# UCL/gp_emulator

Hardware: AMD Instinct MI355X
Metric: test-points/sec for predict(mean+var+grad), N_train=250 D=11 (higher is better)
Workload: dtype f64

## Files before the change

gp_emulator_amd/_lib.py:

```python
import ctypes
import os
import sys
import threading

import numpy as np

from ._dense_numpy import (DAMPINGS, newton_step_numpy, posterior_cov_numpy, prec_rows, prior_propagate_numpy,
                           prior_rows, row_strides, rts_smooth_numpy, _cholesky_inverse_numpy, _mirror_lower)
from ._lut_numpy import MAX_PCS as lut_pc_max_pcs
from ._lut_numpy import lut_pc_prepare_numpy, lut_search_numpy, lut_search_pc_numpy
from ._moments_numpy import rows_arrays as _moments_rows
from ._sobol_numpy import bounds_arrays as _sobol_bounds

HERE = os.path.dirname(os.path.abspath(__file__))
LIB_PATH = os.environ.get("GP_PREDICT_LIB") or os.path.join(HERE, "libgp_predict_hip.so")

GP_F32, GP_F64 = 0, 1
GP_DERIV_DMAJOR, GP_DERIV_ROWMAJOR = 0, 1
GP_DAMP_DIAGONAL, GP_DAMP_IDENTITY = 0, 1
_DAMPING = dict(zip(DAMPINGS, (GP_DAMP_DIAGONAL, GP_DAMP_IDENTITY)))

c_int, c_i64, c_void_p = ctypes.c_int, ctypes.c_int64, ctypes.c_void_p
c_dp = ctypes.POINTER(ctypes.c_double)
c_fp = ctypes.POINTER(ctypes.c_float)
PP = ctypes.POINTER(c_void_p)

SIGNATURES = {
    "gp_last_error_string": (ctypes.c_char_p, []),
    "gp_version_string": (ctypes.c_char_p, []),
    "gp_device_count": (c_int, [ctypes.POINTER(c_int)]),
    "gp_ctx_create": (c_int, [c_int, PP]),
    "gp_ctx_destroy": (c_int, [c_void_p]),
    "gp_ctx_synchronize": (c_int, [c_void_p]),
    "gp_ctx_set_debug_buffer": (c_int, [c_void_p, c_void_p]),
    "gp_ctx_device_info": (c_int, [c_void_p, ctypes.POINTER(c_int), ctypes.POINTER(c_i64),
                                   ctypes.c_char_p, c_int]),
    "gp_predict_wrap_f64": (c_int, [c_void_p] + [c_void_p] * 8 + [c_i64, c_int, c_int, c_int]),
    "gp_predict_wrap_f32": (c_int, [c_void_p] + [c_void_p] * 8 + [c_i64, c_int, c_int, c_int]),
    "gp_predict_rows_f64": (c_int, [c_void_p] + [c_void_p] * 8 + [c_i64, c_int, c_int, c_int]),
    "gp_predict_rows_f32": (c_int, [c_void_p] + [c_void_p] * 8 + [c_i64, c_int, c_int, c_int]),
    "gp_predict_rows_f32_h64": (c_int, [c_void_p] + [c_void_p] * 8 + [c_i64, c_int, c_int, c_int]),
    "gp_model_create_f64": (c_int, [c_void_p] + [c_void_p] * 4 + [c_int, c_int, c_int, PP]),
    "gp_model_create_f32": (c_int, [c_void_p] + [c_void_p] * 4 + [c_int, c_int, c_int, PP]),
    "gp_model_create_f32_h64": (c_int, [c_void_p] + [c_void_p] * 4 + [c_int, c_int, c_int, PP]),
    "gp_batch_create_f32_h64": (c_int, [c_void_p, c_int] + [c_void_p] * 4 + [c_int, c_int, c_int, PP]),
    "gp_batch_create_f64": (c_int, [c_void_p, c_int] + [c_void_p] * 4 + [c_int, c_int, c_int, PP]),
    "gp_batch_create_f32": (c_int, [c_void_p, c_int] + [c_void_p] * 4 + [c_int, c_int, c_int, PP]),
    "gp_model_emulators": (c_int, [c_void_p, ctypes.POINTER(c_int)]),
    "gp_model_destroy": (c_int, [c_void_p]),
    "gp_model_info": (c_int, [c_void_p] + [ctypes.POINTER(c_int)] * 5),
    "gp_predict_device": (c_int, [c_void_p, c_void_p, c_void_p, c_void_p, c_void_p, c_void_p,
                                  c_i64, c_int]),
    "gp_predict_host": (c_int, [c_void_p, c_void_p, c_int, c_void_p, c_void_p, c_void_p, c_void_p,
                                c_i64, c_int, c_i64]),
    "gp_predict_mean_grad_device": (c_int, [c_void_p, c_void_p, c_void_p, c_void_p, c_void_p, c_i64, c_int]),
    "gp_predict_var_grad_device": (c_int, [c_void_p, c_void_p, c_void_p, c_void_p, c_void_p, c_i64, c_int]),
    "gp_model_var_grad_bytes": (c_int, [c_void_p, ctypes.POINTER(c_i64)]),
    "gp_predict_mean_grad_host": (c_int, [c_void_p, c_void_p, c_int, c_void_p, c_void_p, c_void_p,
                                          c_i64, c_int, c_i64]),
    "gp_ctx_host_threads": (c_int, [c_void_p, ctypes.POINTER(c_int)]),
    "gp_device_numa_node": (c_int, [c_int, ctypes.POINTER(c_int)]),
    "gp_kernel_ksteps": (c_int, [c_int, c_int, ctypes.POINTER(c_int)]),
    "gp_hessian_device": (c_int, [c_void_p, c_void_p, c_void_p, c_void_p, c_i64]),
    "gp_hessian_host": (c_int, [c_void_p, c_void_p, c_void_p, c_void_p, c_i64]),
    "gp_hessian_weighted_device": (c_int, [c_void_p, c_void_p, c_void_p, c_void_p, c_void_p, c_i64]),
    "gp_hessian_weighted_host": (c_int, [c_void_p, c_void_p, c_int, c_void_p, c_void_p, c_void_p, c_i64]),
    "gp_band_misfit_device": (c_int, [c_void_p, c_void_p, c_void_p, c_void_p, c_i64, c_i64, c_void_p, c_i64, c_i64,
                                      c_void_p, c_void_p, c_void_p, c_void_p, c_void_p, c_i64]),
    "gp_band_misfit_unc_device": (c_int, [c_void_p, c_void_p, c_void_p, c_void_p, c_i64, c_i64, c_void_p, c_i64, c_i64,
                                          c_void_p, c_void_p, c_void_p, c_void_p, c_void_p, c_i64]),
    "gp_band_misfit_host": (c_int, [c_void_p, c_void_p, c_int, c_void_p, c_void_p, c_i64, c_i64, c_void_p, c_i64, c_i64,
                                    c_void_p, c_void_p, c_void_p, c_void_p, c_void_p, c_i64]),
    "gp_newton_step_device": (c_int, [c_void_p, c_int] + [c_void_p] * 4 + [c_int] + [c_void_p] * 7 + [c_i64, c_int]),
    "gp_lm_update_device": (c_int, [c_void_p, c_int] + [c_void_p] * 14 + [ctypes.c_double] * 6 + [c_i64, c_int]),
    "gp_posterior_cov_device": (c_int, [c_void_p, c_int] + [c_void_p] * 5 + [c_i64, c_int]),
    "gp_newton_step_rows_device": (c_int, [c_void_p, c_int] + [c_void_p] * 4 + [c_int] + [c_void_p] * 7 + [c_i64, c_int, c_i64, c_i64]),
    "gp_lm_update_rows_device": (c_int, [c_void_p, c_int] + [c_void_p] * 14 + [ctypes.c_double] * 6 + [c_i64, c_int, c_i64, c_i64]),
    "gp_posterior_cov_rows_device": (c_int, [c_void_p, c_int] + [c_void_p] * 5 + [c_i64, c_int, c_i64]),
    "gp_prior_propagate_device": (c_int, [c_void_p, c_int, c_void_p, c_void_p, c_i64, c_void_p, c_i64, c_void_p, c_void_p, c_i64, c_int]),
    "gp_rts_smooth_device": (c_int, [c_void_p, c_int, c_void_p, c_void_p, c_i64, c_void_p, c_i64] + [c_void_p] * 9 + [c_i64, c_int]),
    "gp_lut_search_device": (c_int, [c_void_p, c_int, c_void_p, c_i64, c_i64, c_void_p, c_void_p, c_i64, c_i64, c_void_p,
                                     c_i64, c_i64, c_void_p, c_void_p, c_i64, c_i64, c_int, c_int, c_int]),
    "gp_lut_search_geometry": (c_int, [ctypes.POINTER(c_int)] * 3),
    "gp_lut_search_pc_device": (c_int, [c_void_p, c_int, c_void_p, c_i64, c_i64] + [c_void_p] * 5 + [c_i64] + [c_void_p] * 3
                                + [c_i64, c_i64, c_int, c_int, c_int]),
    "gp_lut_search_pc_geometry": (c_int, [c_int, c_int] + [ctypes.POINTER(c_int)] * 4),
    "gp_mv_lut_prepare_device": (c_int, [c_void_p, c_int, c_void_p, c_void_p, c_i64, c_void_p, c_i64, c_void_p, c_i64]
                                 + [c_void_p] * 4 + [c_i64, c_int, c_int]),
    "gp_hessian_f64": (c_int, [c_void_p] + [c_void_p] * 5 + [c_i64, c_int, c_int, c_int]),
    "gp_hessian_f32": (c_int, [c_void_p] + [c_void_p] * 5 + [c_i64, c_int, c_int, c_int]),
    "gp_reconstruct_device": (c_int, [c_void_p, c_int, c_void_p, c_void_p, c_void_p, c_i64, c_int, c_int]),
    "gp_hessian_host_h64": (c_int, [c_void_p, c_void_p, c_void_p, c_void_p, c_i64]),
    "gp_mv_predict_host": (c_int, [c_void_p, c_void_p, c_void_p, c_void_p, c_i64, c_int, c_void_p, c_void_p]),
    "gp_content_digest": (ctypes.c_uint64, [c_void_p, c_void_p, c_int]),
    "gp_mv_predict_host_checked": (c_int, [c_void_p, c_void_p, c_void_p, c_void_p, c_i64, c_int, c_void_p, c_void_p,
                                           c_void_p, c_void_p, c_int, ctypes.c_uint64]),
    "gp_mv_misfit_device": (c_int, [c_void_p, c_int, c_void_p, c_void_p, c_void_p, c_void_p, c_i64, c_void_p, c_i64,
                                    c_void_p, c_void_p, c_void_p, c_i64, c_int, c_int, c_int]),
    "gp_mv_gauss_newton_device": (c_int, [c_void_p, c_int, c_void_p, c_void_p, c_void_p, c_i64, c_int, c_int]),
    "gp_mv_weight_gram_device": (c_int, [c_void_p, c_int, c_void_p, c_void_p, c_i64, c_void_p, c_i64, c_int, c_int]),
    "gp_mv_gauss_newton_rows_device": (c_int, [c_void_p, c_int, c_void_p, c_void_p, c_i64, c_void_p, c_i64, c_int, c_int]),
    "gp_mv_misfit_unc_device": (c_int, [c_void_p, c_int, c_void_p, c_void_p, c_void_p, c_i64] + [c_void_p] * 8
                                + [c_i64, c_int, c_int]),
    "gp_mv_misfit_host": (c_int, [c_void_p, c_void_p, c_void_p, c_void_p, c_i64, c_void_p, c_i64, c_void_p, c_i64,
                                  c_void_p, c_i64, c_int, c_void_p]),
    "gp_mv_misfit_host_checked": (c_int, [c_void_p, c_void_p, c_void_p, c_void_p, c_i64, c_void_p, c_i64, c_void_p, c_i64,
                                          c_void_p, c_i64, c_int, c_void_p, c_void_p, c_void_p, c_int, ctypes.c_uint64]),
    "gp_frag_index": (c_int, [c_int, c_int, c_int, c_int]),
    "gp_likelihood_batch_f64": (c_int, [c_void_p, c_int, c_void_p, c_void_p, c_void_p, c_int, c_int,
                                        c_int, c_void_p, c_void_p, c_void_p, c_void_p]),
    "gp_sobol_batch_f64": (c_int, [c_void_p, c_int, c_void_p, c_void_p, c_void_p, c_int, c_int, c_int, c_void_p, c_void_p,
                                   c_int, c_void_p, c_void_p, c_void_p]),
    "gp_moments_batch_f64": (c_int, [c_void_p, c_int, c_void_p, c_void_p, c_void_p, c_void_p, c_int, c_int, c_i64, c_void_p,
                                     c_void_p, c_int, c_void_p, c_void_p, c_void_p, c_void_p, c_void_p, c_void_p]),
    "gp_pack_sizes": (c_int, [c_int, c_int, c_int, ctypes.POINTER(c_int), ctypes.POINTER(c_int),
                              ctypes.POINTER(c_i64), ctypes.POINTER(c_i64)]),
    "gp_launch_plan": (c_int, [c_int, c_int, c_int, c_int, c_int, c_i64, c_int, c_int, c_int, ctypes.POINTER(c_int),
                               ctypes.POINTER(c_i64), ctypes.POINTER(c_int), ctypes.POINTER(c_i64),
                               ctypes.POINTER(c_int), ctypes.POINTER(c_int)]),
    "gp_pack_model_f64": (c_int, [c_void_p] * 4 + [c_int, c_int, c_int] + [c_void_p] * 4),
    "gp_pack_model_f32": (c_int, [c_void_p] * 4 + [c_int, c_int, c_int] + [c_void_p] * 4),
    "gp_pinned_alloc": (c_int, [c_void_p, c_i64, PP]),
    "gp_pinned_free": (c_int, [c_void_p, c_void_p]),
    "gp_malloc": (c_int, [c_void_p, c_i64, PP]),
    "gp_free": (c_int, [c_void_p, c_void_p]),
    "gp_memcpy_h2d": (c_int, [c_void_p, c_void_p, c_void_p, c_i64]),
    "gp_memcpy_d2h": (c_int, [c_void_p, c_void_p, c_void_p, c_i64]),
    "gp_memset": (c_int, [c_void_p, c_void_p, c_int, c_i64]),
    "gp_event_create": (c_int, [c_void_p, PP]),
    "gp_event_destroy": (c_int, [c_void_p]),
    "gp_event_record": (c_int, [c_void_p, c_void_p]),
    "gp_event_elapsed_ms": (c_int, [c_void_p, c_void_p, ctypes.POINTER(ctypes.c_float)]),
}


class GpuPredictUnavailable(RuntimeError):
    """The HIP library is missing or unusable.  Never caught inside this package."""


class GpuPredictError(RuntimeError):
    """A C-ABI call returned a non-zero status."""


_lib = None
_lock = threading.Lock()


def load():
    global _lib
    with _lock:
        if _lib is not None:
            return _lib
        if not os.path.exists(LIB_PATH):
            raise GpuPredictUnavailable(
                "%s not built; run `python -m gp_emulator_amd.build` (needs hipcc). "
                "There is no CPU fallback for is_gpu=True." % LIB_PATH)
        try:
            lib = ctypes.CDLL(LIB_PATH)
        except OSError as e:
            raise GpuPredictUnavailable("cannot load %s: %s" % (LIB_PATH, e))
        for name, (res, args) in SIGNATURES.items():
            fn = getattr(lib, name)
            fn.restype = res
            fn.argtypes = args
        _lib = lib
        return lib


def check(rc, what=""):
    if rc != 0:
        msg = load().gp_last_error_string().decode("utf-8", "replace")
        raise GpuPredictError("%s failed (status %d): %s" % (what or "gp call", rc, msg))


GP_STALE = 1


class HostBlocks:

    def __init__(self, arrays):
        self.arrays = list(arrays)
        self.ids = tuple(id(a) for a in arrays)
        self._bufs = {}
        src = []
        for i, a in enumerate(self.arrays):
            if isinstance(a, np.ndarray) and a.flags.c_contiguous:
                src.append(a)
            else:
                self._bufs[i] = np.array(a, order="C", copy=True)
                src.append(self._bufs[i])
        self.n = len(src)
        self.ptrs = (c_void_p * self.n)(*[a.ctypes.data for a in src])
        self.lens = (c_i64 * self.n)(*[a.nbytes for a in src])
        self.expected = self.digest()

    def same_arrays(self, arrays):
        return self.ids == tuple(id(a) for a in arrays)

    def refresh(self):
        for i, buf in self._bufs.items():
            a = np.asarray(self.arrays[i])
            if a.shape == buf.shape and a.dtype == buf.dtype:
                np.copyto(buf, a)
            else:
                buf.view(np.uint8)[...] = 0xA5
        return self

    def digest(self):
        self.refresh()
        return int(load().gp_content_digest(self.ptrs, self.lens, self.n))

    def unchanged(self):
        return self.digest() == self.expected


def device_count():
    n = c_int(0)
    rc = load().gp_device_count(ctypes.byref(n))
    if rc != 0:
        return 0
    return n.value


def _ptr(a):
    return a.ctypes.data_as(c_void_p)


def _dtype_code(dtype):
    return GP_F64 if np.dtype(dtype) == np.float64 else GP_F32


def precision_dtype(precision):
    dt = np.dtype(precision)
    if dt not in (np.dtype(np.float32), np.dtype(np.float64)):
        raise TypeError("precision must be float32 or float64, got %r" % (precision,))
    return dt


def _out_array(a, shape, dtype, pool=None):
    if a is None:
        return pool.take(shape, dtype) if pool is not None else np.empty(shape, dtype)
    if (not isinstance(a, np.ndarray) or a.dtype != dtype or a.shape != shape
            or not a.flags["C_CONTIGUOUS"] or not a.flags["WRITEABLE"]):
        raise ValueError("out must be a writeable C-contiguous %s %s array" % (shape, np.dtype(dtype)))
    return a


def _device_dtype(precision, a):
    return np.dtype(precision if precision is not None else (np.float32 if a.dtype == np.float32 else np.float64))


def _matrix_rows(A, precision):
    A = np.asarray(A)
    if A.ndim != 3 or A.shape[1] != A.shape[2]:
        raise ValueError("A must be (n_rows, n_inputs, n_inputs)")
    return A, _device_dtype(precision, A), A.shape[0], A.shape[1]


def device_numa_cpus(device=0):
    node = c_int(-1)
    if load().gp_device_numa_node(int(device), ctypes.byref(node)) != 0 or node.value < 0:
        return set()
    try:
        text = open("/sys/devices/system/node/node%d/cpulist" % node.value).read().strip()
    except OSError:
        return set()
    cpus = set()
    for part in text.split(","):
        if part:
            a, _, b = part.partition("-")
            cpus.update(range(int(a), int(b or a) + 1))
    return cpus & set(os.sched_getaffinity(0))


def bind_near_device(device=0):
    cpus = device_numa_cpus(device)
    if cpus:
        os.sched_setaffinity(0, cpus)
    return cpus


class OutputPool:

    def __init__(self, max_item=256 << 20, max_total=1 << 30):
        self.max_item, self.max_total = max_item, max_total
        self.items = []

    def take(self, shape, dtype):
        dtype = np.dtype(dtype)
        nbytes = int(np.prod(shape, dtype=np.int64)) * dtype.itemsize
        if nbytes < (1 << 20) or nbytes > self.max_item:
            return np.empty(shape, dtype)
        base = None
        for cand in self.items:
            if cand.nbytes == nbytes and sys.getrefcount(cand) == 3:
                base = cand
                break
        cand = None
        if base is None:
            base = np.empty(nbytes, np.uint8)
            self.items.append(base)
            total = sum(b.nbytes for b in self.items)
            for free_first in (True, False):
                i = 0
                while total > self.max_total and i < len(self.items):
                    b = self.items[i]
                    if b is not base and (not free_first or sys.getrefcount(b) == 3):
                        total -= b.nbytes
                        del self.items[i]
                    else:
                        i += 1
                b = None
        return base.view(dtype).reshape(shape)


class Scratch(object):

    def __init__(self, ctx, dt):
        self.ctx, self.dt, self.held = ctx, dt, []

    def up(self, a):
        if a is None:
            return None
        self.held.append(self.ctx.to_device(np.ascontiguousarray(a, dtype=self.dt)))
        return self.held[-1]

    def alloc(self, nbytes):
        self.held.append(self.ctx.malloc(max(1, nbytes)))
        return self.held[-1]

    def __enter__(self):
        return self

    def __exit__(self, *exc):
        held, self.held = self.held, []
        for p in held:
            self.ctx.free(p)


def _download(ctx, dptr, shape, dtype):
    return np.array(ctx.to_host(dptr, shape, dtype))


class Context:

    def __init__(self, device=0):
        self.lib = load()
        h = c_void_p()
        rc = self.lib.gp_ctx_create(int(device), ctypes.byref(h))
        if rc != 0:
            msg = self.lib.gp_last_error_string().decode("utf-8", "replace")
            raise GpuPredictUnavailable("no usable GPU context on device %d: %s" % (device, msg))
        self.h = h
        self.device = int(device)
        self.out_pool = OutputPool()

    def pinned_empty(self, shape, dtype=np.float64):
        import weakref
        dtype = np.dtype(dtype)
        n = int(np.prod(shape, dtype=np.int64))
        nbytes = max(1, n * dtype.itemsize)
        ptr = c_void_p()
        check(self.lib.gp_pinned_alloc(self.h, nbytes, ctypes.byref(ptr)), "gp_pinned_alloc")
        buf = (ctypes.c_char * nbytes).from_address(ptr.value)
        arr = np.frombuffer(buf, dtype=np.uint8, count=n * dtype.itemsize).view(dtype).reshape(shape)
        lib, h, addr = self.lib, self.h, ptr.value
        weakref.finalize(buf, lambda: lib.gp_pinned_free(h, c_void_p(addr)))
        return arr

    def close(self):
        if getattr(self, "h", None):
            self.lib.gp_ctx_destroy(self.h)
            self.h = None

    __del__ = close

    def synchronize(self):
        check(self.lib.gp_ctx_synchronize(self.h), "gp_ctx_synchronize")

    def device_info(self):
        cu, mem = c_int(0), c_i64(0)
        name = ctypes.create_string_buffer(256)
        check(self.lib.gp_ctx_device_info(self.h, ctypes.byref(cu), ctypes.byref(mem), name, 256))
        return dict(compute_units=cu.value, hbm_bytes=mem.value, name=name.value.decode())

    def host_threads(self):
        n = c_int(0)
        check(self.lib.gp_ctx_host_threads(self.h, ctypes.byref(n)), "gp_ctx_host_threads")
        return n.value

    def malloc(self, nbytes):
        p = c_void_p()
        check(self.lib.gp_malloc(self.h, int(nbytes), ctypes.byref(p)), "gp_malloc")
        return p

    def free(self, p):
        check(self.lib.gp_free(self.h, p), "gp_free")

    def to_device(self, arr):
        arr = np.ascontiguousarray(arr)
        p = self.malloc(max(arr.nbytes, 1))
        if arr.nbytes:
            check(self.lib.gp_memcpy_h2d(self.h, p, _ptr(arr), arr.nbytes), "gp_memcpy_h2d")
        return p

    def h2d(self, dptr, arr):
        arr = np.ascontiguousarray(arr)
        check(self.lib.gp_memcpy_h2d(self.h, dptr, _ptr(arr), arr.nbytes), "gp_memcpy_h2d")

    def to_host(self, dptr, shape, dtype):
        out = self.out_pool.take(shape, dtype)
        if out.nbytes:
            check(self.lib.gp_memcpy_d2h(self.h, _ptr(out), dptr, out.nbytes), "gp_memcpy_d2h")
        return out

    def to_host_at(self, dptr, offset_bytes, shape, dtype):
        out = np.empty(shape, dtype=dtype)
        src = c_void_p(dptr.value + int(offset_bytes))
        check(self.lib.gp_memcpy_d2h(self.h, _ptr(out), src, out.nbytes), "gp_memcpy_d2h")
        return out

    def reconstruct_device(self, dtype, d_basis, d_coef, d_out, n_rows, n_pcs, n_bands):
        check(self.lib.gp_reconstruct_device(self.h, _dtype_code(dtype), d_basis, d_coef, d_out, int(n_rows),
                                             int(n_pcs), int(n_bands)), "gp_reconstruct_device")

    def mv_misfit_device(self, dtype, d_basis, d_mu, d_deriv, d_obs, obs_stride, d_weights, weights_stride,
                         d_cost, d_coef, d_grad, n_rows, n_pcs, n_bands, n_inputs):
        check(self.lib.gp_mv_misfit_device(self.h, _dtype_code(dtype), d_basis, d_mu, d_deriv, d_obs, int(obs_stride), d_weights,
                                           int(weights_stride), d_cost, d_coef, d_grad, int(n_rows), int(n_pcs),
                                           int(n_bands), int(n_inputs)), "gp_mv_misfit_device")

    def mv_gauss_newton_device(self, dtype, d_deriv, d_A, d_gn, n_rows, n_pcs, n_inputs):
        check(self.lib.gp_mv_gauss_newton_device(self.h, _dtype_code(dtype), d_deriv, d_A, d_gn, int(n_rows), int(n_pcs),
                                                 int(n_inputs)), "gp_mv_gauss_newton_device")

    def mv_weight_gram_device(self, dtype, d_basis, d_weights, weights_stride, d_gram, n_rows, n_pcs, n_bands):
        check(self.lib.gp_mv_weight_gram_device(self.h, _dtype_code(dtype), d_basis, d_weights, int(weights_stride), d_gram,
                                                int(n_rows), int(n_pcs), int(n_bands)), "gp_mv_weight_gram_device")

    def mv_gauss_newton_rows_device(self, dtype, d_deriv, d_gram, gram_stride, d_gn, n_rows, n_pcs, n_inputs):
        check(self.lib.gp_mv_gauss_newton_rows_device(self.h, _dtype_code(dtype), d_deriv, d_gram, int(gram_stride), d_gn, int(n_rows),
                                                      int(n_pcs), int(n_inputs)), "gp_mv_gauss_newton_rows_device")

    def mv_misfit_unc_device(self, dtype, d_cost0, d_coef, d_gram, gram_stride, d_var, d_deriv, d_dvar, d_cost, d_grad,
                             d_gn, n_rows, n_pcs, n_inputs, d_ceff=None, d_geff=None):
        check(self.lib.gp_mv_misfit_unc_device(self.h, _dtype_code(dtype), d_cost0, d_coef, d_gram, int(gram_stride), d_var,
                                               d_deriv, d_dvar, d_cost, d_grad, d_gn, d_ceff, d_geff, int(n_rows), int(n_pcs),
                                               int(n_inputs)), "gp_mv_misfit_unc_device")

    def newton_step_device(self, dtype, d_x, d_grad, d_A, d_lambda, d_step, d_trial, d_status, n_rows, n_inputs,
                           damping="diagonal", d_prior_mean=None, d_prior_prec=None, d_lo=None, d_hi=None):
        check(self.lib.gp_newton_step_device(self.h, _dtype_code(dtype), d_x, d_grad, d_A, d_lambda, _DAMPING[damping], d_prior_mean,
                                             d_prior_prec, d_lo, d_hi, d_step, d_trial, d_status, int(n_rows),
                                             int(n_inputs)), "gp_newton_step_device")

    def lm_update_device(self, dtype, d_x, d_trial, d_cost, d_cost_trial, d_grad, d_grad_trial, d_A, d_A_trial, d_lambda,
                         d_status, d_state, d_accepted, n_rows, n_inputs, d_prior_mean=None, d_prior_prec=None,
                         down=1.0 / 3.0, up=4.0, lambda_min=1e-12, lambda_max=1e12, ftol=1e-10, xtol=0.0):
        check(self.lib.gp_lm_update_device(self.h, _dtype_code(dtype), d_x, d_trial, d_cost, d_cost_trial, d_grad, d_grad_trial, d_A,
                                           d_A_trial, d_lambda, d_status, d_state, d_accepted, d_prior_mean, d_prior_prec,
                                           float(down), float(up), float(lambda_min), float(lambda_max), float(ftol),
                                           float(xtol), int(n_rows), int(n_inputs)), "gp_lm_update_device")

    def posterior_cov_device(self, dtype, d_A, d_prior_prec, d_cov, d_sigma, d_status, n_rows, n_inputs):
        check(self.lib.gp_posterior_cov_device(self.h, _dtype_code(dtype), d_A, d_prior_prec, d_cov, d_sigma, d_status, int(n_rows),
                                               int(n_inputs)), "gp_posterior_cov_device")

    def newton_step_rows_device(self, dtype, d_x, d_grad, d_A, d_lambda, d_step, d_trial, d_status, n_rows, n_inputs,
                                damping="diagonal", d_prior_mean=None, d_prior_prec=None, d_lo=None, d_hi=None,
                                prior_mean_stride=0, prior_prec_stride=0):
        check(self.lib.gp_newton_step_rows_device(self.h, _dtype_code(dtype), d_x, d_grad, d_A, d_lambda, _DAMPING[damping], d_prior_mean,
                                                  d_prior_prec, d_lo, d_hi, d_step, d_trial, d_status, int(n_rows),
                                                  int(n_inputs), int(prior_mean_stride), int(prior_prec_stride)),
              "gp_newton_step_rows_device")

    def lm_update_rows_device(self, dtype, d_x, d_trial, d_cost, d_cost_trial, d_grad, d_grad_trial, d_A, d_A_trial,
                              d_lambda, d_status, d_state, d_accepted, n_rows, n_inputs, d_prior_mean=None,
                              d_prior_prec=None, down=1.0 / 3.0, up=4.0, lambda_min=1e-12, lambda_max=1e12, ftol=1e-10,
                              xtol=0.0, prior_mean_stride=0, prior_prec_stride=0):
        check(self.lib.gp_lm_update_rows_device(self.h, _dtype_code(dtype), d_x, d_trial, d_cost, d_cost_trial, d_grad, d_grad_trial, d_A,
                                                d_A_trial, d_lambda, d_status, d_state, d_accepted, d_prior_mean,
                                                d_prior_prec, float(down), float(up), float(lambda_min), float(lambda_max),
                                                float(ftol), float(xtol), int(n_rows), int(n_inputs),
                                                int(prior_mean_stride), int(prior_prec_stride)), "gp_lm_update_rows_device")

    def posterior_cov_rows_device(self, dtype, d_A, d_prior_prec, d_cov, d_sigma, d_status, n_rows, n_inputs,
                                  prior_prec_stride=0):
        check(self.lib.gp_posterior_cov_rows_device(self.h, _dtype_code(dtype), d_A, d_prior_prec, d_cov, d_sigma, d_status, int(n_rows),
                                                    int(n_inputs), int(prior_prec_stride)), "gp_posterior_cov_rows_device")

    def prior_propagate_device(self, dtype, d_A, d_prior_prec, prior_prec_stride, d_noise, noise_stride, d_next_prec,
                               d_status, n_rows, n_inputs):
        check(self.lib.gp_prior_propagate_device(self.h, _dtype_code(dtype), d_A, d_prior_prec, int(prior_prec_stride), d_noise,
                                                 int(noise_stride), d_next_prec, d_status, int(n_rows), int(n_inputs)),
              "gp_prior_propagate_device")

    def prior_propagate(self, A, prior_prec, noise, precision=None, is_gpu=True):
        if not is_gpu:
            return prior_propagate_numpy(A, prior_prec, noise)
        A, dt, M, D = _matrix_rows(A, precision)
        P = prec_rows(prior_prec, M, D, dt) if prior_prec is not None else None
        Q = prec_rows(noise, M, D, dt)
        with Scratch(self, dt) as scratch:
            d_A, d_P, d_Q = scratch.up(A), scratch.up(P), scratch.up(Q)
            d_next, d_status = scratch.alloc(M * D * D * dt.itemsize), scratch.alloc(M * 4)
            self.prior_propagate_device(dt, d_A, d_P, row_strides(None, P)[1], d_Q, row_strides(None, Q)[1], d_next, d_status,
                                        M, D)
            return _download(self, d_next, (M, D, D), dt), _download(self, d_status, (M,), np.int32)

    def rts_smooth_device(self, dtype, d_A, d_prior_prec, prior_prec_stride, d_noise, noise_stride, d_x, d_x_next,
                          d_cov_next, d_lo, d_hi, d_x_smooth, d_cov_smooth, d_sigma_smooth, d_status, n_rows, n_inputs):
        check(self.lib.gp_rts_smooth_device(self.h, _dtype_code(dtype), d_A, d_prior_prec, int(prior_prec_stride), d_noise,
                                            int(noise_stride), d_x, d_x_next, d_cov_next, d_lo, d_hi, d_x_smooth,
                                            d_cov_smooth, d_sigma_smooth, d_status, int(n_rows), int(n_inputs)),
              "gp_rts_smooth_device")

    def rts_smooth(self, A, prior_prec, noise, x, x_next, cov_next, bounds=None, precision=None, is_gpu=True):
        if not is_gpu:
            return rts_smooth_numpy(A, prior_prec, noise, x, x_next, cov_next, bounds)
        A, dt, M, D = _matrix_rows(A, precision)
        P = prec_rows(prior_prec, M, D, dt) if prior_prec is not None else None
        Q = prec_rows(noise, M, D, dt)
        ins = [A, P, Q, np.reshape(x, (M, D)), np.reshape(x_next, (M, D)), np.reshape(cov_next, (M, D, D))]
        ins += [np.reshape(b, D) for b in bounds] if bounds is not None else [None, None]
        with Scratch(self, dt) as scratch:
            d_A, d_P, d_Q, d_x, d_xn, d_cn, d_lo, d_hi = [scratch.up(a) for a in ins]
            isz = dt.itemsize
            d_xs, d_cov, d_sigma, d_status = (scratch.alloc(M * D * isz), scratch.alloc(M * D * D * isz),
                                              scratch.alloc(M * D * isz), scratch.alloc(M * 4))
            self.rts_smooth_device(dt, d_A, d_P, row_strides(None, P)[1], d_Q, row_strides(None, Q)[1], d_x, d_xn, d_cn,
                                   d_lo, d_hi, d_xs, d_cov, d_sigma, d_status, M, D)
            return (_download(self, d_xs, (M, D), dt), _download(self, d_cov, (M, D, D), dt),
                    _download(self, d_sigma, (M, D), dt), _download(self, d_status, (M,), np.int32))

    def posterior_cov(self, A, prior_prec=None, precision=None, is_gpu=True):
        if not is_gpu:
            return posterior_cov_numpy(A, prior_prec)
        A, dt, M, D = _matrix_rows(A, precision)
        P = prec_rows(prior_prec, M, D, dt) if prior_prec is not None else None
        with Scratch(self, dt) as scratch:
            d_A, d_P = scratch.up(A), scratch.up(P)
            d_cov, d_sigma, d_status = scratch.alloc(M * D * D * dt.itemsize), scratch.alloc(M * D * dt.itemsize), scratch.alloc(M * 4)
            if P is not None and P.ndim == 3:
                self.posterior_cov_rows_device(dt, d_A, d_P, d_cov, d_sigma, d_status, M, D, D * D)
            else:
                self.posterior_cov_device(dt, d_A, d_P, d_cov, d_sigma, d_status, M, D)
            return (_download(self, d_cov, (M, D, D), dt), _download(self, d_sigma, (M, D), dt),
                    _download(self, d_status, (M,), np.int32))

    def newton_step(self, x, grad, A, lam, damping="diagonal", prior=None, bounds=None, precision=None, is_gpu=True):
        if not is_gpu:
            return newton_step_numpy(x, grad, A, lam, damping, prior, bounds)
        if damping not in _DAMPING:
            raise ValueError("damping must be 'diagonal' or 'identity'")
        x = np.asarray(x)
        if x.ndim != 2:
            raise ValueError("x must be (n_rows, n_inputs)")
        dt = _device_dtype(precision, x)
        M, D = x.shape
        host = [x, np.reshape(grad, (M, D)), np.reshape(A, (M, D, D)), np.broadcast_to(np.asarray(lam, dtype=dt), (M,))]
        host += list(prior_rows(prior, M, D, dt)) if prior is not None else [None, None]
        strides = row_strides(host[4], host[5])
        host += [np.reshape(b, D) for b in bounds] if bounds is not None else [None, None]
        with Scratch(self, dt) as scratch:
            d_x, d_grad, d_A, d_lam, d_x0, d_P, d_lo, d_hi = [scratch.up(a) for a in host]
            d_step, d_trial, d_status = scratch.alloc(M * D * dt.itemsize), scratch.alloc(M * D * dt.itemsize), scratch.alloc(M * 4)
            if any(strides):
                self.newton_step_rows_device(dt, d_x, d_grad, d_A, d_lam, d_step, d_trial, d_status, M, D, damping, d_x0, d_P,
                                             d_lo, d_hi, *strides)
            else:
                self.newton_step_device(dt, d_x, d_grad, d_A, d_lam, d_step, d_trial, d_status, M, D, damping, d_x0, d_P,
                                        d_lo, d_hi)
            return (_download(self, d_step, (M, D), dt), _download(self, d_trial, (M, D), dt),
                    _download(self, d_status, (M,), np.int32))

    def lut_search_device(self, dtype, d_table, table_strides, d_offset, d_obs, obs_strides, d_weights, w_strides, d_index,
                          d_cost, n_rows, n_candidates, n_terms, n_best, n_slices=0):
        check(self.lib.gp_lut_search_device(self.h, _dtype_code(dtype), d_table, int(table_strides[0]), int(table_strides[1]),
                                            d_offset, d_obs, int(obs_strides[0]), int(obs_strides[1]), d_weights,
                                            int(w_strides[0]), int(w_strides[1]), d_index, d_cost, int(n_rows),
                                            int(n_candidates), int(n_terms), int(n_best), int(n_slices)),
              "gp_lut_search_device")

    def lut_search_pc_device(self, dtype, d_table, table_strides, d_offset, d_c0, d_j0, d_g0, d_gram, gram_stride, d_status,
                             d_index, d_cost, n_rows, n_candidates, n_pcs, n_best, n_slices=0):
        check(self.lib.gp_lut_search_pc_device(self.h, _dtype_code(dtype), d_table, int(table_strides[0]), int(table_strides[1]),
                                               d_offset, d_c0, d_j0, d_g0, d_gram, int(gram_stride), d_status, d_index, d_cost,
                                               int(n_rows), int(n_candidates), int(n_pcs), int(n_best), int(n_slices)),
              "gp_lut_search_pc_device")

    def mv_lut_prepare_device(self, dtype, d_basis, d_obs, obs_stride, d_weights, weights_stride, d_gram, gram_stride,
                              d_c0, d_j0, d_g0, d_status, n_rows, n_pcs, n_bands):
        check(self.lib.gp_mv_lut_prepare_device(self.h, _dtype_code(dtype), d_basis, d_obs, int(obs_stride), d_weights,
                                                int(weights_stride), d_gram, int(gram_stride), d_c0, d_j0, d_g0, d_status,
                                                int(n_rows), int(n_pcs), int(n_bands)), "gp_mv_lut_prepare_device")

    def lut_search(self, table, obs, weights=None, offset=None, n_best=1, precision=None, is_gpu=True, n_slices=0):
        if not is_gpu:
            return lut_search_numpy(table, obs, weights, offset, n_best)
        table = np.asarray(table)
        if table.ndim != 2:
            raise ValueError("table must be (n_candidates, n_terms)")
        dt = _device_dtype(precision, table)
        L, K = table.shape
        obs = np.asarray(obs)
        weights = None if weights is None else np.asarray(weights)
        for name, a in (("obs", obs), ("weights", weights)):
            if a is not None and (a.ndim not in (1, 2) or a.shape[-1] != K):
                raise ValueError("%s must be (%d,) or (n_rows, %d), got %s" % (name, K, K, a.shape))
        rows = [a.shape[0] for a in (obs, weights) if a is not None and a.ndim == 2]
        M = rows[0] if rows else 1
        if any(r != M for r in rows):
            raise ValueError("obs and weights disagree on the number of rows")

        def strides(a):
            return (1, K) if a.ndim == 2 else (1, 0)
        with Scratch(self, dt) as scratch:
            d_t, d_o, d_w, d_a = scratch.up(table), scratch.up(obs), scratch.up(weights), scratch.up(offset)
            d_i, d_c = scratch.alloc(M * n_best * 4), scratch.alloc(M * n_best * dt.itemsize)
            self.lut_search_device(dt, d_t, (1, K), d_a, d_o, strides(obs), d_w, strides(weights) if weights is not None else (0, 0),
                                   d_i, d_c, M, L, K, n_best, n_slices)
            return _download(self, d_i, (M, n_best), np.int32), _download(self, d_c, (M, n_best), dt)

    def likelihood_batch(self, thetas, inputs, targets, want_inverse=False):
        thetas = np.ascontiguousarray(np.atleast_2d(thetas), dtype=np.float64)
        inputs = np.ascontiguousarray(inputs, dtype=np.float64)
        targets = np.ascontiguousarray(targets, dtype=np.float64)
        E, N, D = thetas.shape[0], inputs.shape[0], inputs.shape[1]
        if thetas.shape[1] != D + 2:
            raise ValueError("theta needs n_inputs + 2 entries")
        shared = targets.ndim == 1
        if targets.shape[-1] != N or (not shared and targets.shape[0] != E):
            raise ValueError("targets must be (n_train,) or (n_sets, n_train)")
        cost = np.empty(E)
        grad = np.empty((E, D + 2))
        invQ = np.empty((E, N, N)) if want_inverse else None
        invQt = np.empty((E, N)) if want_inverse else None
        check(self.lib.gp_likelihood_batch_f64(
            self.h, E, _ptr(thetas), _ptr(inputs), _ptr(targets), int(shared), N, D, _ptr(cost),
            _ptr(grad), _ptr(invQ) if want_inverse else None,
            _ptr(invQt) if want_inverse else None), "gp_likelihood_batch_f64")
        return (cost, grad, invQ, invQt) if want_inverse else (cost, grad)

    def sobol_batch(self, expX, inputs, invQt, lo, hi, pairs=None):
        expX = np.ascontiguousarray(np.atleast_2d(expX), dtype=np.float64)
        inputs = np.ascontiguousarray(inputs, dtype=np.float64)
        invQt = np.ascontiguousarray(np.atleast_2d(invQt), dtype=np.float64)
        if inputs.ndim != 2:
            raise ValueError("inputs must be (n_train, n_inputs)")
        (N, D), E = inputs.shape, expX.shape[0]
        if expX.shape != (E, D + 2):
            raise ValueError("expX must be (n_emulators, n_inputs + 2), got %s" % (expX.shape,))
        if invQt.shape != (E, N):
            raise ValueError("invQt must be (n_emulators, n_train), got %s" % (invQt.shape,))
        lo, hi, boxed = _sobol_bounds(lo, hi, D)
        if pairs is not None:
            pairs = np.ascontiguousarray(pairs, dtype=np.int32)
            if pairs.ndim != 2 or pairs.shape[1] != 2:
                raise ValueError("pairs must be (n_pairs, 2)")
        B, P = lo.shape[0], E if pairs is None else pairs.shape[0]
        mean, cov = np.empty((B, E)), np.empty((B, P, 1 + 2 * D))
        check(self.lib.gp_sobol_batch_f64(self.h, E, _ptr(expX), _ptr(inputs), _ptr(invQt), N, D, B, _ptr(lo), _ptr(hi), P,
                                          None if pairs is None else _ptr(pairs), _ptr(mean), _ptr(cov)),
              "gp_sobol_batch_f64")
        return (mean, cov) if boxed else (mean[0], cov[0])

    def moments_batch(self, expX, inputs, invQt, invQ, mean_in, cov_in, pairs=None):
        expX = np.ascontiguousarray(np.atleast_2d(expX), dtype=np.float64)
        inputs = np.ascontiguousarray(inputs, dtype=np.float64)
        invQt = np.ascontiguousarray(np.atleast_2d(invQt), dtype=np.float64)
        if inputs.ndim != 2:
            raise ValueError("inputs must be (n_train, n_inputs)")
        (N, D), E = inputs.shape, expX.shape[0]
        if expX.shape != (E, D + 2):
            raise ValueError("expX must be (n_emulators, n_inputs + 2), got %s" % (expX.shape,))
        if invQt.shape != (E, N):
            raise ValueError("invQt must be (n_emulators, n_train), got %s" % (invQt.shape,))
        if invQ is not None:
            invQ = np.ascontiguousarray(invQ, dtype=np.float64)
            if invQ.size != E * N * N:
                raise ValueError("invQ must be (n_emulators, n_train, n_train), got %s" % (invQ.shape,))
        m, S = _moments_rows(mean_in, cov_in, D)
        if pairs is not None:
            pairs = np.ascontiguousarray(pairs, dtype=np.int32)
            if pairs.ndim != 2 or pairs.shape[1] != 2:
                raise ValueError("pairs must be (n_pairs, 2)")
        M, P = m.shape[0], E if pairs is None else pairs.shape[0]
        mean, egrad, cov = np.empty((M, E)), np.empty((M, E, D)), np.empty((M, P))
        evar = None if invQ is None else np.empty((M, E))
        info = np.empty(M, np.int32)
        check(self.lib.gp_moments_batch_f64(self.h, E, _ptr(expX), _ptr(inputs), _ptr(invQt),
                                            None if invQ is None else _ptr(invQ), N, D, M, _ptr(m), _ptr(S), P,
                                            None if pairs is None else _ptr(pairs), _ptr(mean), _ptr(egrad), _ptr(cov),
                                            None if evar is None else _ptr(evar), _ptr(info)), "gp_moments_batch_f64")
        return mean, egrad, cov, evar, info

    def event(self):
        e = c_void_p()
        check(self.lib.gp_event_create(self.h, ctypes.byref(e)), "gp_event_create")
        return e

    def record(self, ev):
        check(self.lib.gp_event_record(self.h, ev), "gp_event_record")

    def elapsed_ms(self, e0, e1):
        ms = ctypes.c_float(0)
        check(self.lib.gp_event_elapsed_ms(e0, e1, ctypes.byref(ms)), "gp_event_elapsed_ms")
        return ms.value

    def event_destroy(self, ev):
        self.lib.gp_event_destroy(ev)


class Model:

    n_emulators = None
    _create = "gp_model_create"

    def __init__(self, ctx, expX, inputs, invQt, invQ, precision=np.float64):
        self.ctx = ctx
        self.dtype = precision_dtype(precision)
        inputs = np.ascontiguousarray(inputs, dtype=np.float64)
        if inputs.ndim != 2:
            raise ValueError("inputs must be (n_train, n_inputs)")
        self.n_train, self.n_inputs = inputs.shape
        expX = np.ascontiguousarray(expX, dtype=np.float64)
        invQt = np.ascontiguousarray(invQt, dtype=np.float64)
        if invQ is not None:
            invQ = np.ascontiguousarray(invQ, dtype=np.float64)
        expX, invQt, lead = self._emulator_constants(expX, invQt, invQ)
        fn = getattr(ctx.lib, self._create + ("_f64" if self.dtype == np.float64 else "_f32_h64"))
        h = c_void_p()
        check(fn(ctx.h, *lead, _ptr(expX), _ptr(inputs), _ptr(invQt), _ptr(invQ) if invQ is not None else None,
                 self.n_train, self.n_inputs, expX.shape[-1], ctypes.byref(h)), self._create)
        self.h = h

    def _emulator_constants(self, expX, invQt, invQ):
        expX, invQt = expX.ravel(), invQt.ravel()
        if invQt.size != self.n_train:
            raise ValueError("invQt size does not match n_train")
        if invQ is not None and invQ.size != self.n_train ** 2:
            raise ValueError("invQ size does not match n_train")
        return expX, invQt, ()

    def __enter__(self):
        return self

    def __exit__(self, *exc):
        self.close()

    def info(self):
        v = [c_int(0) for _ in range(5)]
        check(self.ctx.lib.gp_model_info(self.h, *[ctypes.byref(x) for x in v]))
        nk = c_int(0)
        check(self.ctx.lib.gp_kernel_ksteps(v[1].value, v[2].value, ctypes.byref(nk)))
        vg = c_i64(0)
        check(self.ctx.lib.gp_model_var_grad_bytes(self.h, ctypes.byref(vg)))
        return dict(dtype=v[0].value, n_train=v[1].value, n_inputs=v[2].value,
                    kernel_d=v[3].value, kernel_nb=v[4].value, kernel_nk=nk.value, var_grad_bytes=vg.value)

    def predict_device(self, d_testing, d_mu, d_var, d_deriv, n_predict,
                       deriv_layout=GP_DERIV_ROWMAJOR):
        check(self.ctx.lib.gp_predict_device(self.ctx.h, self.h, d_testing, d_mu, d_var, d_deriv,
                                             int(n_predict), int(deriv_layout)), "gp_predict_device")

    def predict(self, testing, deriv_layout=GP_DERIV_ROWMAJOR, out=None, max_block_rows=0):
        testing, outs = self._host_call(testing, deriv_layout, out, with_var=True)
        mu, var, deriv = outs
        M = testing.shape[0]
        if M:
            check(self.ctx.lib.gp_predict_host(
                self.ctx.h, self.h, _dtype_code(testing.dtype), _ptr(testing), _ptr(mu),
                _ptr(var), _ptr(deriv), M, int(deriv_layout), int(max_block_rows)), "gp_predict_host")
        return mu, var, deriv

    def predict_mean_grad_device(self, d_testing, d_mu, d_deriv, n_predict, deriv_layout=GP_DERIV_ROWMAJOR):
        check(self.ctx.lib.gp_predict_mean_grad_device(self.ctx.h, self.h, d_testing, d_mu, d_deriv,
                                                       int(n_predict), int(deriv_layout)),
              "gp_predict_mean_grad_device")

    def predict_mean_grad(self, testing, deriv_layout=GP_DERIV_ROWMAJOR, out=None, max_block_rows=0):
        testing, outs = self._host_call(testing, deriv_layout, out, with_var=False)
        mu, deriv = outs
        M = testing.shape[0]
        if M:
            check(self.ctx.lib.gp_predict_mean_grad_host(
                self.ctx.h, self.h, _dtype_code(testing.dtype), _ptr(testing),
                _ptr(mu), _ptr(deriv), M, int(deriv_layout), int(max_block_rows)), "gp_predict_mean_grad_host")
        return mu, deriv

    def predict_var_grad_device(self, d_testing, d_var, d_dvar, n_predict, deriv_layout=GP_DERIV_ROWMAJOR):
        check(self.ctx.lib.gp_predict_var_grad_device(self.ctx.h, self.h, d_testing, d_var, d_dvar,
                                                      int(n_predict), int(deriv_layout)), "gp_predict_var_grad_device")

    VAR_GRAD_BLOCK_ROWS = 1 << 20

    def predict_var_grad(self, testing, deriv_layout=GP_DERIV_ROWMAJOR, out=None):
        testing = np.ascontiguousarray(testing, dtype=self.dtype)
        if testing.ndim != 2 or testing.shape[1] != self.n_inputs:
            raise ValueError("testing must be (n_predict, %d)" % self.n_inputs)
        M, D = testing.shape
        E = self.n_emulators
        lead, ne = (() if E is None else (E,)), (E or 1)
        row_major = deriv_layout == GP_DERIV_ROWMAJOR
        shapes = (lead + (M,), lead + ((M, D) if row_major else (D, M)))
        var, dvar = (None, None) if out is None else out
        if out is not None and (var is None or dvar is None):
            raise ValueError("out must hold 2 arrays")
        var, dvar = (_out_array(a, shape, self.dtype) for a, shape in zip((var, dvar), shapes))
        v2, d3 = var.reshape(ne, M), dvar.reshape((ne, M, D) if row_major else (ne, D, M))
        isz = self.dtype.itemsize
        for lo in range(0, M, self.VAR_GRAD_BLOCK_ROWS):
            n = min(self.VAR_GRAD_BLOCK_ROWS, M - lo)
            with Scratch(self.ctx, self.dtype) as scratch:
                d_t = scratch.up(testing[lo:lo + n])
                d_var, d_dvar = scratch.alloc(ne * n * isz), scratch.alloc(ne * n * D * isz)
                self.predict_var_grad_device(d_t, d_var, d_dvar, n, deriv_layout)
                v2[:, lo:lo + n] = _download(self.ctx, d_var, (ne, n), self.dtype)
                blk = _download(self.ctx, d_dvar, (ne, n, D) if row_major else (ne, D, n), self.dtype)
                if row_major:
                    d3[:, lo:lo + n] = blk
                else:
                    d3[:, :, lo:lo + n] = blk
        return var, dvar

    def _host_call(self, testing, deriv_layout, out, with_var):
        testing = np.asarray(testing)
        if testing.dtype != np.float64 or self.dtype == np.float64:
            testing = np.ascontiguousarray(testing, dtype=self.dtype)
        else:
            testing = np.ascontiguousarray(testing)
        hdt = testing.dtype
        if testing.ndim != 2:
            raise ValueError("testing must be (n_predict, n_inputs)")
        M, D = testing.shape
        if D != self.n_inputs:
            raise ValueError("testing has %d columns, model has %d inputs" % (D, self.n_inputs))
        E = self.n_emulators
        lead = () if E is None else (E,)
        dshape = lead + ((M, D) if deriv_layout == GP_DERIV_ROWMAJOR else (D, M))
        nv = 2 if with_var else 1
        shapes = (lead + (M,),) * nv + (dshape,)
        if out is None:
            n_e = (E or 1) * M
            flat = self.ctx.out_pool.take((n_e * (nv + D),), hdt)
            outs = tuple(flat[k * n_e:(k + 1) * n_e].reshape(lead + (M,)) for k in range(nv))
            outs += (flat[nv * n_e:].reshape(dshape),)
        else:
            outs = tuple(out)
            if len(outs) != nv + 1 or any(a is None for a in outs):
                raise ValueError("out must hold %d arrays" % (nv + 1))
            outs = tuple(_out_array(a, shape, hdt) for a, shape in zip(outs, shapes))
        return testing, outs

    def hessian_device(self, d_testing, d_hess, n_predict):
        check(self.ctx.lib.gp_hessian_device(self.ctx.h, self.h, d_testing, d_hess,
                                             int(n_predict)), "gp_hessian_device")

    def _hessian_rows(self, testing):
        testing = np.asarray(testing)
        h64 = testing.dtype == np.float64 and self.dtype != np.float64
        hdt = np.dtype(np.float64) if h64 else self.dtype
        testing = np.ascontiguousarray(testing, dtype=hdt)
        if testing.ndim != 2 or testing.shape[1] != self.n_inputs:
            raise ValueError("testing must be (n_predict, %d)" % self.n_inputs)
        return testing, hdt, h64

    def hessian(self, testing, out=None):
        testing, hdt, h64 = self._hessian_rows(testing)
        M, D = testing.shape
        lead = () if self.n_emulators is None else (self.n_emulators,)
        hess = _out_array(out, lead + (M, D, D), hdt, self.ctx.out_pool)
        if M:
            fn = self.ctx.lib.gp_hessian_host_h64 if h64 else self.ctx.lib.gp_hessian_host
            check(fn(self.ctx.h, self.h, _ptr(testing), _ptr(hess), M), "gp_hessian_host")
        return hess

    def close(self):
        if getattr(self, "h", None):
            self.ctx.lib.gp_model_destroy(self.h)
            self.h = None

    __del__ = close


class BatchModel(Model):

    _create = "gp_batch_create"

    def _emulator_constants(self, expX, invQt, invQ):
        if expX.ndim != 2:
            raise ValueError("expX must be (n_emulators, theta_size)")
        self.n_emulators = E = expX.shape[0]
        if invQt.shape != (E, self.n_train) or (invQ is not None and invQ.shape != (E, self.n_train, self.n_train)):
            raise ValueError("invQt must be (E, N) and invQ (E, N, N)")
        return expX, invQt, (E,)

    def hessian_weighted_device(self, d_testing, d_weights, d_out, n_predict):
        check(self.ctx.lib.gp_hessian_weighted_device(self.ctx.h, self.h, d_testing, d_weights, d_out,
                                                      int(n_predict)), "gp_hessian_weighted_device")

    def hessian_weighted(self, testing, weights, out=None):
        testing, hdt, _ = self._hessian_rows(testing)
        M, D = testing.shape
        weights = np.ascontiguousarray(weights, dtype=hdt)
        if weights.shape != (self.n_emulators, M):
            raise ValueError("weights must be (%d, %d)" % (self.n_emulators, M))
        res = _out_array(out, (M, D, D), hdt, self.ctx.out_pool)
        if M:
            check(self.ctx.lib.gp_hessian_weighted_host(
                self.ctx.h, self.h, _dtype_code(hdt), _ptr(testing), _ptr(weights),
                _ptr(res), M), "gp_hessian_weighted_host")
        return res

    def misfit_device(self, d_testing, d_obs, obs_strides, d_weights, w_strides, d_cost, d_grad, n_rows,
                      d_wr=None, d_gn=None, d_hess=None):
        ws = w_strides if d_weights is not None else (0, 0)
        check(self.ctx.lib.gp_band_misfit_device(
            self.ctx.h, self.h, d_testing, d_obs, int(obs_strides[0]), int(obs_strides[1]), d_weights, int(ws[0]),
            int(ws[1]), d_cost, d_grad, d_wr, d_gn, d_hess, int(n_rows)), "gp_band_misfit_device")

    def _em_array(self, a, M, hdt, name):
        a = np.ascontiguousarray(a, dtype=hdt)
        E = self.n_emulators
        if a.shape == (E,):
            return a, (1, 0)
        if a.shape == (E, M):
            return a, (M, 1)
        raise ValueError("%s must be (%d,) or (%d, %d), got %s" % (name, E, E, M, a.shape))

    def misfit(self, testing, obs, weights=None, second_order=None, return_residual=False):
        if second_order not in (None, "gauss_newton", "full"):
            raise ValueError("second_order must be None, 'gauss_newton' or 'full'")
        testing, hdt, _ = self._hessian_rows(testing)
        M, D = testing.shape
        obs, os_ = self._em_array(obs, M, hdt, "obs")
        ws = (0, 0)
        if weights is not None:
            weights, ws = self._em_array(weights, M, hdt, "weights")
        cost, grad = np.empty((M,), hdt), np.empty((M, D), hdt)
        second = np.empty((M, D, D), hdt) if second_order else None
        wr = np.empty((self.n_emulators, M), hdt) if return_residual else None
        if M:
            check(self.ctx.lib.gp_band_misfit_host(
                self.ctx.h, self.h, _dtype_code(hdt), _ptr(testing), _ptr(obs), os_[0], os_[1],
                _ptr(weights) if weights is not None else None, ws[0], ws[1], _ptr(cost), _ptr(grad),
                _ptr(wr) if wr is not None else None, _ptr(second) if second_order == "gauss_newton" else None,
                _ptr(second) if second_order == "full" else None, M), "gp_band_misfit_host")
        out = (cost, grad)
        if second_order:
            out += (second,)
        if return_residual:
            out += (wr,)
        return out

    def misfit_unc_device(self, d_testing, d_obs, obs_strides, d_weights, w_strides, d_cost, d_grad, n_rows,
                          d_wr=None, d_weff=None, d_gn=None):
        ws = w_strides if d_weights is not None else (0, 0)
        check(self.ctx.lib.gp_band_misfit_unc_device(
            self.ctx.h, self.h, d_testing, d_obs, int(obs_strides[0]), int(obs_strides[1]), d_weights, int(ws[0]),
            int(ws[1]), d_cost, d_grad, d_wr, d_weff, d_gn, int(n_rows)), "gp_band_misfit_unc_device")

    MISFIT_UNC_BLOCK_ROWS = 1 << 20

    def misfit_unc(self, testing, obs, weights=None, second_order=None, return_residual=False):
        if second_order == "full":
            raise ValueError("second_order='full' needs the Hessian of the variance: not available with the emulator variance")
        if second_order not in (None, "gauss_newton"):
            raise ValueError("second_order must be None or 'gauss_newton'")
        dt = self.dtype
        testing = np.ascontiguousarray(testing, dtype=dt)
        if testing.ndim != 2 or testing.shape[1] != self.n_inputs:
            raise ValueError("testing must be (n_rows, %d)" % self.n_inputs)
        M, D = testing.shape
        E = self.n_emulators
        obs, os_ = self._em_array(obs, M, dt, "obs")
        if weights is not None:
            weights, ws = self._em_array(weights, M, dt, "weights")
        cost, grad = np.empty((M,), dt), np.empty((M, D), dt)
        gn = np.empty((M, D, D), dt) if second_order else None
        wr, weff = (np.empty((E, M), dt), np.empty((E, M), dt)) if return_residual else (None, None)
        isz = dt.itemsize

        def rows_of(a, strides, lo, n):
            return (a, strides) if strides[1] == 0 else (a[:, lo:lo + n], (n, 1))
        for lo in range(0, M, self.MISFIT_UNC_BLOCK_ROWS):
            n = min(self.MISFIT_UNC_BLOCK_ROWS, M - lo)
            with Scratch(self.ctx, dt) as scratch:
                d_t = scratch.up(testing[lo:lo + n])
                o_blk, o_st = rows_of(obs, os_, lo, n)
                d_o = scratch.up(o_blk)
                d_w, w_st = None, (0, 0)
                if weights is not None:
                    w_blk, w_st = rows_of(weights, ws, lo, n)
                    d_w = scratch.up(w_blk)
                d_c, d_g = scratch.alloc(n * isz), scratch.alloc(n * D * isz)
                d_gn = scratch.alloc(n * D * D * isz) if second_order else None
                d_wr, d_we = (scratch.alloc(E * n * isz), scratch.alloc(E * n * isz)) if return_residual else (None, None)
                self.misfit_unc_device(d_t, d_o, o_st, d_w, w_st, d_c, d_g, n, d_wr=d_wr, d_weff=d_we, d_gn=d_gn)
                cost[lo:lo + n] = _download(self.ctx, d_c, (n,), dt)
                grad[lo:lo + n] = _download(self.ctx, d_g, (n, D), dt)
                if second_order:
                    gn[lo:lo + n] = _download(self.ctx, d_gn, (n, D, D), dt)
                if return_residual:
                    wr[:, lo:lo + n] = _download(self.ctx, d_wr, (E, n), dt)
                    weff[:, lo:lo + n] = _download(self.ctx, d_we, (E, n), dt)
        out = (cost, grad)
        if second_order:
            out += (gn,)
        if return_residual:
            out += (wr, weff)
        return out


GP_OP_PREDICT, GP_OP_MEAN_GRAD, GP_OP_HESSIAN, GP_OP_RECONSTRUCT, GP_OP_MISFIT, GP_OP_MV_GRAM, GP_OP_VAR_GRAD = 0, 1, 2, 3, 4, 5, 6
GP_OP_LUT_SEARCH = 7
GP_OP_LUT_SEARCH_PC = 8
GP_OP_SOBOL = 9
GP_OP_MOMENTS = 10
PLAN_KERNELS = {1: "predict_few", 2: "predict", 3: "generic", 4: "hessian_valu", 5: "hessian_win_kl3",
                6: "hessian_win_kl4", 7: "hessian_win_direct", 8: "reconstruct_narrow", 9: "reconstruct_wide",
                10: "misfit", 11: "mv_gram", 12: "var_grad", 13: "lut_search", 14: "lut_search_pc", 15: "sobol",
                16: "moments"}
_PLAN_OPS = {"predict": GP_OP_PREDICT, "mean_grad": GP_OP_MEAN_GRAD, "hessian": GP_OP_HESSIAN,
             "reconstruct": GP_OP_RECONSTRUCT, "misfit": GP_OP_MISFIT, "mv_gram": GP_OP_MV_GRAM, "var_grad": GP_OP_VAR_GRAD,
             "lut_search": GP_OP_LUT_SEARCH, "lut_search_pc": GP_OP_LUT_SEARCH_PC, "sobol": GP_OP_SOBOL,
             "moments": GP_OP_MOMENTS}


def lut_search_geometry():
    r, t, c = c_int(0), c_int(0), c_int(0)
    check(load().gp_lut_search_geometry(ctypes.byref(r), ctypes.byref(t), ctypes.byref(c)), "gp_lut_search_geometry")
    return dict(rows_per_item=r.value, candidate_tile=t.value, term_chunk=c.value)


def lut_search_pc_geometry(n_pcs, precision=np.float64):
    r, t, pp, w = c_int(0), c_int(0), c_int(0), c_int(0)
    check(load().gp_lut_search_pc_geometry(_dtype_code(precision), int(n_pcs), ctypes.byref(r), ctypes.byref(t),
                                           ctypes.byref(pp), ctypes.byref(w)), "gp_lut_search_pc_geometry")
    return dict(rows_per_item=r.value, candidate_tile=t.value, padded_pcs=pp.value, workgroups_per_cu=w.value)


def launch_plan(op, precision, n_rows, n_train=0, n_inputs=0, n_emulators=1, n_pcs=0, n_bands=0,
                compute_units=256, aligned16=True, n_terms=0, n_candidates=0):
    code = _PLAN_OPS[op]
    recon = code in (GP_OP_RECONSTRUCT, GP_OP_MISFIT, GP_OP_MV_GRAM, GP_OP_LUT_SEARCH, GP_OP_LUT_SEARCH_PC)
    if code == GP_OP_LUT_SEARCH:
        n_pcs, n_bands = n_terms, n_candidates
    if code == GP_OP_LUT_SEARCH_PC:
        n_bands = n_candidates
    k, wg, rwg, rpi = c_int(0), c_int(0), c_int(0), c_int(0)
    items, ritems = c_i64(0), c_i64(0)
    check(load().gp_launch_plan(
        code, _dtype_code(precision), int(n_train), int(n_pcs if recon else n_inputs),
        int(n_emulators), int(n_rows), int(n_bands if recon else 0), int(compute_units), int(bool(aligned16)),
        ctypes.byref(k), ctypes.byref(items), ctypes.byref(wg), ctypes.byref(ritems), ctypes.byref(rwg),
        ctypes.byref(rpi)), "gp_launch_plan")
    if code == GP_OP_LUT_SEARCH:
        geo = lut_search_geometry()
        return dict(kernel=PLAN_KERNELS[k.value], rows_per_item=rpi.value, items=items.value, workgroups=wg.value,
                    rest_items=0, rest_workgroups=0, slices=ritems.value, candidate_tile=geo["candidate_tile"],
                    term_chunk=geo["term_chunk"])
    if code == GP_OP_LUT_SEARCH_PC:
        geo = lut_search_pc_geometry(n_pcs, precision)
        return dict(kernel=PLAN_KERNELS[k.value], rows_per_item=rpi.value, items=items.value, workgroups=wg.value,
                    rest_items=0, rest_workgroups=0, slices=ritems.value, candidate_tile=geo["candidate_tile"],
                    padded_pcs=geo["padded_pcs"], workgroups_per_cu=geo["workgroups_per_cu"])
    return dict(kernel=PLAN_KERNELS[k.value], rows_per_item=rpi.value, items=items.value, workgroups=wg.value,
                rest_items=ritems.value, rest_workgroups=rwg.value)


def pack_model(expX, inputs, invQt, invQ, precision=np.float64):
    lib = load()
    dt = np.dtype(precision)
    inputs = np.ascontiguousarray(inputs, dtype=dt)
    N, D = inputs.shape
    expX = np.ascontiguousarray(expX, dtype=dt).ravel()
    invQt = np.ascontiguousarray(invQt, dtype=dt).ravel()
    invQ = np.ascontiguousarray(invQ, dtype=dt)
    kd, knb, xl, fl = c_int(0), c_int(0), c_i64(0), c_i64(0)
    check(lib.gp_pack_sizes(_dtype_code(dt), N, D, ctypes.byref(kd),
                            ctypes.byref(knb), ctypes.byref(xl), ctypes.byref(fl)), "gp_pack_sizes")
    xa = np.zeros(xl.value, dt)
    fr = np.zeros(fl.value, dt)
    sd = np.zeros(2 * kd.value + 1, dt)
    b = np.zeros(1, dt)
    fn = lib.gp_pack_model_f64 if dt == np.float64 else lib.gp_pack_model_f32
    check(fn(_ptr(expX), _ptr(inputs), _ptr(invQt), _ptr(invQ), N, D, expX.size,
             _ptr(xa), _ptr(fr), _ptr(sd), _ptr(b)), "gp_pack_model")
    nk = c_int(0)
    check(lib.gp_kernel_ksteps(N, D, ctypes.byref(nk)), "gp_kernel_ksteps")
    return dict(xa=xa, frags=fr, sd=sd[:kd.value], centre=sd[kd.value:2 * kd.value], b=b[0],
                kernel_d=kd.value, kernel_nb=knb.value, kernel_nk=nk.value)


_tls = threading.local()


_default_device = [None]


def set_default_device(device):
    _default_device[0] = int(device)


def default_device():
    if _default_device[0] is None:
        _default_device[0] = int(os.environ.get("GP_DEVICE", "0"))
    return _default_device[0]


def default_context(device=None):
    device = default_device() if device is None else int(device)
    d = getattr(_tls, "ctx", None)
    if d is None:
        d = _tls.ctx = {}
    c = d.get(device)
    if c is None:
        c = d[device] = Context(device)
    return c
```

gp_emulator_amd/csrc/gp_ctx.hip:

```cpp
#include "gp_host.hpp"

#include <cstdarg>
#include <cstdio>

#include "gp_launchers.hpp"
#include "gp_train_args.hpp"

static thread_local char g_err[512] = "";

int fail(int code, const char* fmt, ...) {
  va_list ap;
  va_start(ap, fmt);
  vsnprintf(g_err, sizeof(g_err), fmt, ap);
  va_end(ap);
  return code;
}

int check_call(const gp_ctx* ctx, const gp_model* model, int64_t n) {
  if (!ctx || !model) return fail(GP_ERR_INVALID, "null context or model");
  if (n < 0) return fail(GP_ERR_INVALID, "n_predict < 0");
  return GP_OK;
}
int check_layout(int deriv_layout) {
  if (deriv_layout == GP_DERIV_DMAJOR || deriv_layout == GP_DERIV_ROWMAJOR) return GP_OK;
  return fail(GP_ERR_INVALID, "bad deriv_layout %d", deriv_layout);
}
int check_hessian_inputs(int n_inputs) {
  if (n_inputs <= GP_MAX_KERNEL_D) return GP_OK;
  return fail(GP_ERR_UNSUPPORTED, "hessian kernels are compiled for n_inputs <= %d", GP_MAX_KERNEL_D);
}
int check_model(const gp_ctx* ctx, const gp_model* model, int needs) {
  if (model->device != ctx->device) return fail(GP_ERR_INVALID, "model lives on device %d, context on %d", model->device, ctx->device);
  if ((needs & kNeedVariance) && !model->d_frags) return fail(GP_ERR_INVALID, "model was created without invQ: no variance operand");
  if (needs & kNeedHessian) return check_hessian_inputs(model->n_inputs);
  return GP_OK;
}

int ensure_scratch(gp_ctx* ctx, size_t bytes) {
  if (ctx->scratch_bytes >= bytes) return GP_OK;
  if (ctx->scratch) {
    HIP_TRY(hipStreamSynchronize(ctx->stream));
    HIP_TRY(hipFree(ctx->scratch));
    ctx->scratch = nullptr;
    ctx->scratch_bytes = 0;
  }
  HIP_TRY(hipMalloc(&ctx->scratch, bytes));
  ctx->scratch_bytes = bytes;
  return GP_OK;
}

extern "C" {

const char* gp_last_error_string(void) { return g_err; }
const char* gp_version_string(void) { return "gp_predict_hip 0.1 (gfx950)"; }

int gp_device_count(int* count) {
  if (!count) return fail(GP_ERR_INVALID, "null pointer");
  int n = 0;
  hipError_t e = hipGetDeviceCount(&n);
  if (e != hipSuccess) {
    *count = 0;
    return fail(GP_ERR_NO_DEVICE, "hipGetDeviceCount: %s", hipGetErrorString(e));
  }
  *count = n;
  return GP_OK;
}

int gp_ctx_create(int device, gp_ctx** out) {
  if (!out) return fail(GP_ERR_INVALID, "null pointer");
  *out = nullptr;
  int n = 0;
  int rc = gp_device_count(&n);
  if (rc) return rc;
  if (n <= 0) return fail(GP_ERR_NO_DEVICE, "no HIP device visible");
  if (device < 0 || device >= n) return fail(GP_ERR_INVALID, "device %d out of range [0,%d)", device, n);
  HIP_TRY(hipSetDevice(device));
  hipDeviceProp_t prop;
  HIP_TRY(hipGetDeviceProperties(&prop, device));
  gp_ctx* c = new (std::nothrow) gp_ctx();
  if (!c) return fail(GP_ERR_NOMEM, "out of host memory");
  c->device = device;
  c->compute_units = prop.multiProcessorCount;
  c->scratch = nullptr;
  c->scratch_bytes = 0;
  c->dbg = nullptr;
  hipError_t e = hipStreamCreateWithFlags(&c->stream, hipStreamNonBlocking);
  if (e != hipSuccess) {
    delete c;
    return fail(GP_ERR_HIP, "hipStreamCreate: %s", hipGetErrorString(e));
  }
  e = hipMalloc((void**)&c->tickets, 4 * kTicketSlots * sizeof(unsigned));
  if (e == hipSuccess) e = hipMemset(c->tickets, 0, 4 * kTicketSlots * sizeof(unsigned));
  if (e != hipSuccess) {
    if (c->tickets) (void)hipFree(c->tickets);
    (void)hipStreamDestroy(c->stream);
    delete c;
    return fail(GP_ERR_HIP, "context item counters: %s", hipGetErrorString(e));
  }
  *out = c;
  return GP_OK;
}

int gp_ctx_destroy(gp_ctx* ctx) {
  if (!ctx) return GP_OK;
  (void)hipSetDevice(ctx->device);
  (void)hipStreamSynchronize(ctx->stream);
  for (auto& c : ctx->cache)
    if (c.model) gp_model_destroy(c.model);
  if (ctx->scratch) (void)hipFree(ctx->scratch);
  if (ctx->tickets) (void)hipFree(ctx->tickets);
  gp_pipe& pp = ctx->pipe;
  pp.pool.reset();
  for (int k = 0; k < kPipeSlots; ++k) {
    if (pp.stream[k]) (void)hipStreamSynchronize(pp.stream[k]);
    if (pp.stage_in[k]) (void)hipHostFree(pp.stage_in[k]);
    if (pp.stage_out[k]) (void)hipHostFree(pp.stage_out[k]);
    if (pp.dev[k]) (void)hipFree(pp.dev[k]);
    if (pp.done[k]) (void)hipEventDestroy(pp.done[k]);
    if (pp.in_there[k]) (void)hipEventDestroy(pp.in_there[k]);
    if (pp.computed[k]) (void)hipEventDestroy(pp.computed[k]);
    if (pp.stream[k]) (void)hipStreamDestroy(pp.stream[k]);
  }
  if (pp.up) { (void)hipStreamSynchronize(pp.up); (void)hipStreamDestroy(pp.up); }
  if (pp.down) { (void)hipStreamSynchronize(pp.down); (void)hipStreamDestroy(pp.down); }
  (void)hipStreamDestroy(ctx->stream);
  delete ctx;
  return GP_OK;
}

int gp_ctx_set_debug_buffer(gp_ctx* ctx, void* d_buffer) {
  if (!ctx) return fail(GP_ERR_INVALID, "null context");
  ctx->dbg = d_buffer;
  return GP_OK;
}

int gp_ctx_synchronize(gp_ctx* ctx) {
  if (!ctx) return fail(GP_ERR_INVALID, "null context");
  HIP_TRY(hipSetDevice(ctx->device));
  HIP_TRY(hipStreamSynchronize(ctx->stream));
  return GP_OK;
}

int gp_ctx_device_info(gp_ctx* ctx, int* compute_units, int64_t* hbm_bytes, char* name, int name_len) {
  if (!ctx) return fail(GP_ERR_INVALID, "null context");
  hipDeviceProp_t prop;
  HIP_TRY(hipGetDeviceProperties(&prop, ctx->device));
  if (compute_units) *compute_units = prop.multiProcessorCount;
  if (hbm_bytes) *hbm_bytes = (int64_t)prop.totalGlobalMem;
  if (name && name_len > 0) {
    snprintf(name, name_len, "%s (%s)", prop.name, prop.gcnArchName);
  }
  return GP_OK;
}

int gp_likelihood_batch_f64(gp_ctx* ctx, int n_sets, const double* theta, const double* inputs,
                            const double* targets, int targets_shared, int n_train, int n_inputs,
                            double* cost, double* grad, double* invQ, double* invQt) {
  if (!ctx) return fail(GP_ERR_INVALID, "null context");
  if (!theta || !inputs || !targets || !cost || !grad) return fail(GP_ERR_INVALID, "null pointer");
  if (n_sets <= 0 || n_train <= 0 || n_inputs <= 0) return fail(GP_ERR_INVALID, "bad sizes");
  if (n_train > gpk::tkMaxN || n_inputs > gpk::tkMaxD)
    return fail(GP_ERR_UNSUPPORTED, "likelihood kernel is compiled for n_train <= %d, n_inputs <= %d",
                gpk::tkMaxN, gpk::tkMaxD);
  HIP_TRY(hipSetDevice(ctx->device));
  const size_t E = (size_t)n_sets, N = (size_t)n_train, D = (size_t)n_inputs;
  const size_t n_theta = E * (D + 2), n_in = N * D, n_tg = (targets_shared ? 1 : E) * N;
  const size_t n_work = E * N * N, n_qt = E * N, n_cost = E, n_grad = E * (D + 2);
  int rc = ensure_scratch(ctx, sizeof(double) * (n_theta + n_in + n_tg + n_work + n_qt + n_cost + n_grad));
  if (rc) return rc;
  double* d_theta = (double*)ctx->scratch;
  double* d_in = d_theta + n_theta;
  double* d_tg = d_in + n_in;
  double* d_work = d_tg + n_tg;
  double* d_qt = d_work + n_work;
  double* d_cost = d_qt + n_qt;
  double* d_grad = d_cost + n_cost;
  hipStream_t st = ctx->stream;
  HIP_TRY(hipMemcpyAsync(d_theta, theta, sizeof(double) * n_theta, hipMemcpyHostToDevice, st));
  HIP_TRY(hipMemcpyAsync(d_in, inputs, sizeof(double) * n_in, hipMemcpyHostToDevice, st));
  HIP_TRY(hipMemcpyAsync(d_tg, targets, sizeof(double) * n_tg, hipMemcpyHostToDevice, st));
  gpk::TrainArgs a;
  a.theta = d_theta; a.inputs = d_in; a.targets = d_tg;
  a.targets_stride = targets_shared ? 0 : (long long)N;
  a.work = d_work; a.invQt = d_qt; a.cost = d_cost; a.grad = d_grad;
  a.N = n_train; a.D = n_inputs;
  a.full_inverse = invQ != nullptr;
  a.dbg = (unsigned long long*)ctx->dbg;
  hipError_t e = gpk::launch_likelihood(a, n_sets, st);
  if (e != hipSuccess) return fail(GP_ERR_HIP, "likelihood kernel launch: %s", hipGetErrorString(e));
  HIP_TRY(hipMemcpyAsync(cost, d_cost, sizeof(double) * n_cost, hipMemcpyDeviceToHost, st));
  HIP_TRY(hipMemcpyAsync(grad, d_grad, sizeof(double) * n_grad, hipMemcpyDeviceToHost, st));
  if (invQt) HIP_TRY(hipMemcpyAsync(invQt, d_qt, sizeof(double) * n_qt, hipMemcpyDeviceToHost, st));
  if (invQ) HIP_TRY(hipMemcpyAsync(invQ, d_work, sizeof(double) * n_work, hipMemcpyDeviceToHost, st));
  HIP_TRY(hipStreamSynchronize(st));
  return GP_OK;
}

int gp_pinned_alloc(gp_ctx* ctx, int64_t bytes, void** ptr) {
  if (!ctx || !ptr) return fail(GP_ERR_INVALID, "null pointer");
  if (bytes <= 0) return fail(GP_ERR_INVALID, "bytes must be positive");
  HIP_TRY(hipSetDevice(ctx->device));
  hipError_t err = hipSuccess;
  const int dev = ctx->device;
  void* q = nullptr;
  host_pool(ctx).run_on_worker([&] {
    err = hipSetDevice(dev);
    if (err == hipSuccess) err = hipHostMalloc(&q, (size_t)bytes, hipHostMallocDefault);
    if (err == hipSuccess) std::memset(q, 0, (size_t)bytes);
  });
  if (err != hipSuccess) return fail(GP_ERR_HIP, "gp_pinned_alloc(%lld bytes): %s", (long long)bytes, hipGetErrorString(err));
  *ptr = q;
  return GP_OK;
}
int gp_pinned_free(gp_ctx* ctx, void* ptr) {
  if (!ctx) return fail(GP_ERR_INVALID, "null context");
  if (!ptr) return GP_OK;
  HIP_TRY(hipSetDevice(ctx->device));
  HIP_TRY(hipHostFree(ptr));
  return GP_OK;
}
int gp_malloc(gp_ctx* ctx, int64_t bytes, void** dptr) {
  if (!ctx || !dptr) return fail(GP_ERR_INVALID, "null pointer");
  if (bytes <= 0) return fail(GP_ERR_INVALID, "bytes must be positive");
  HIP_TRY(hipSetDevice(ctx->device));
  HIP_TRY(hipMalloc(dptr, (size_t)bytes));
  return GP_OK;
}
int gp_free(gp_ctx* ctx, void* dptr) {
  if (!ctx) return fail(GP_ERR_INVALID, "null context");
  if (!dptr) return GP_OK;
  HIP_TRY(hipSetDevice(ctx->device));
  HIP_TRY(hipFree(dptr));
  return GP_OK;
}
int gp_memcpy_h2d(gp_ctx* ctx, void* dst, const void* src, int64_t bytes) {
  if (!ctx || !dst || !src) return fail(GP_ERR_INVALID, "null pointer");
  HIP_TRY(hipSetDevice(ctx->device));
  HIP_TRY(hipMemcpyAsync(dst, src, (size_t)bytes, hipMemcpyHostToDevice, ctx->stream));
  HIP_TRY(hipStreamSynchronize(ctx->stream));
  return GP_OK;
}
int gp_memcpy_d2h(gp_ctx* ctx, void* dst, const void* src, int64_t bytes) {
  if (!ctx || !dst || !src) return fail(GP_ERR_INVALID, "null pointer");
  HIP_TRY(hipSetDevice(ctx->device));
  HIP_TRY(hipMemcpyAsync(dst, src, (size_t)bytes, hipMemcpyDeviceToHost, ctx->stream));
  HIP_TRY(hipStreamSynchronize(ctx->stream));
  return GP_OK;
}
int gp_memset(gp_ctx* ctx, void* dptr, int value, int64_t bytes) {
  if (!ctx || !dptr) return fail(GP_ERR_INVALID, "null pointer");
  HIP_TRY(hipSetDevice(ctx->device));
  HIP_TRY(hipMemsetAsync(dptr, value, (size_t)bytes, ctx->stream));
  return GP_OK;
}

int gp_event_create(gp_ctx* ctx, gp_event** out) {
  if (!ctx || !out) return fail(GP_ERR_INVALID, "null pointer");
  HIP_TRY(hipSetDevice(ctx->device));
  gp_event* e = new (std::nothrow) gp_event();
  if (!e) return fail(GP_ERR_NOMEM, "out of host memory");
  e->device = ctx->device;
  hipError_t r = hipEventCreate(&e->ev);
  if (r != hipSuccess) {
    delete e;
    return fail(GP_ERR_HIP, "hipEventCreate: %s", hipGetErrorString(r));
  }
  *out = e;
  return GP_OK;
}
int gp_event_destroy(gp_event* ev) {
  if (!ev) return GP_OK;
  (void)hipSetDevice(ev->device);
  (void)hipEventDestroy(ev->ev);
  delete ev;
  return GP_OK;
}
int gp_event_record(gp_ctx* ctx, gp_event* ev) {
  if (!ctx || !ev) return fail(GP_ERR_INVALID, "null pointer");
  HIP_TRY(hipSetDevice(ctx->device));
  HIP_TRY(hipEventRecord(ev->ev, ctx->stream));
  return GP_OK;
}
int gp_event_elapsed_ms(gp_event* start, gp_event* stop, float* ms) {
  if (!start || !stop || !ms) return fail(GP_ERR_INVALID, "null pointer");
  HIP_TRY(hipSetDevice(stop->device));
  HIP_TRY(hipEventSynchronize(stop->ev));
  HIP_TRY(hipEventElapsedTime(ms, start->ev, stop->ev));
  return GP_OK;
}

}
```

gp_emulator_amd/csrc/gp_host_path.hip:

```cpp
#include "gp_host.hpp"

#include <cctype>
#include <chrono>
#include <cstdio>

#include <sched.h>

static int device_numa_node(int device) {
  char bdf[64] = "";
  if (hipDeviceGetPCIBusId(bdf, (int)sizeof(bdf), device) != hipSuccess) return -1;
  for (char* c = bdf; *c; ++c) *c = (char)tolower(*c);
  char path[160];
  snprintf(path, sizeof(path), "/sys/bus/pci/devices/%s/numa_node", bdf);
  FILE* fh = fopen(path, "r");
  if (!fh) return -1;
  int node = -1;
  if (fscanf(fh, "%d", &node) != 1) node = -1;
  fclose(fh);
  return node;
}
static bool node_cpus(int node, cpu_set_t* out) {
  CPU_ZERO(out);
  if (node < 0) return false;
  char path[96];
  snprintf(path, sizeof(path), "/sys/devices/system/node/node%d/cpulist", node);
  FILE* fh = fopen(path, "r");
  if (!fh) return false;
  cpu_set_t allowed;
  CPU_ZERO(&allowed);
  if (sched_getaffinity(0, sizeof(allowed), &allowed) != 0) { fclose(fh); return false; }
  int a, b, n = 0;
  while (fscanf(fh, "%d", &a) == 1) {
    b = a;
    int ch = fgetc(fh);
    if (ch == '-') { if (fscanf(fh, "%d", &b) != 1) break; ch = fgetc(fh); }
    for (int c = a; c <= b && c < CPU_SETSIZE; ++c)
      if (CPU_ISSET(c, &allowed)) { CPU_SET(c, out); ++n; }
    if (ch != ',') break;
  }
  fclose(fh);
  return n > 0;
}

static int host_threads() {
  static int n = [] {
    int avail = 1;
    cpu_set_t set;
    CPU_ZERO(&set);
    if (sched_getaffinity(0, sizeof(set), &set) == 0) avail = CPU_COUNT(&set);
    const char* ev = getenv("GP_HOST_THREADS");
    int v = ev ? atoi(ev) : 8;
    if (v > avail) v = avail;
    return v < 1 ? 1 : (v > 32 ? 32 : v);
  }();
  return n;
}

gph::ThreadPool& host_pool(gp_ctx* ctx) {
  if (!ctx->pipe.pool) {
    cpu_set_t cpus;
    const char* ev = getenv("GP_HOST_PIN");
    const bool pin = (!ev || atoi(ev) != 0) && node_cpus(device_numa_node(ctx->device), &cpus);
    ctx->pipe.pool.reset(new gph::ThreadPool(host_threads(), pin ? &cpus : nullptr));
  }
  return *ctx->pipe.pool;
}

static int ensure_pipe(gp_ctx* ctx, size_t in_bytes, size_t out_bytes, size_t dev_only_bytes = 0) {
  gp_pipe& pp = ctx->pipe;
  if (!pp.ready) {
    for (int k = 0; k < kPipeSlots; ++k) {
      if (!pp.stream[k]) HIP_TRY(hipStreamCreateWithFlags(&pp.stream[k], hipStreamNonBlocking));
      if (!pp.done[k]) HIP_TRY(hipEventCreateWithFlags(&pp.done[k], hipEventDisableTiming));
      if (!pp.in_there[k]) HIP_TRY(hipEventCreateWithFlags(&pp.in_there[k], hipEventDisableTiming));
      if (!pp.computed[k]) HIP_TRY(hipEventCreateWithFlags(&pp.computed[k], hipEventDisableTiming));
    }
    if (!pp.up) HIP_TRY(hipStreamCreateWithFlags(&pp.up, hipStreamNonBlocking));
    if (!pp.down) HIP_TRY(hipStreamCreateWithFlags(&pp.down, hipStreamNonBlocking));
    pp.ready = true;
  }
  auto host_alloc = [&](void** slot, size_t bytes) -> hipError_t {
    hipError_t err = hipSuccess;
    const int dev = ctx->device;
    host_pool(ctx).run_on_worker([&] {
      err = hipSetDevice(dev);
      if (err == hipSuccess) err = hipHostMalloc(slot, bytes, hipHostMallocDefault);
      if (err == hipSuccess) std::memset(*slot, 0, bytes);
    });
    return err;
  };
  if (dev_only_bytes == 0 && pp.stage_in_bytes < in_bytes) {
    pp.stage_in_bytes = 0;
    for (int k = 0; k < kPipeSlots; ++k) {
      if (pp.stage_in[k]) { void* q = pp.stage_in[k]; pp.stage_in[k] = nullptr; HIP_TRY(hipHostFree(q)); }
      HIP_TRY(host_alloc(&pp.stage_in[k], in_bytes));
    }
    pp.stage_in_bytes = in_bytes;
  }
  if (dev_only_bytes == 0 && pp.stage_out_bytes < out_bytes) {
    pp.stage_out_bytes = 0;
    for (int k = 0; k < kPipeSlots; ++k) {
      if (pp.stage_out[k]) { void* q = pp.stage_out[k]; pp.stage_out[k] = nullptr; HIP_TRY(hipHostFree(q)); }
      HIP_TRY(host_alloc(&pp.stage_out[k], out_bytes));
    }
    pp.stage_out_bytes = out_bytes;
  }
  const size_t dev_need = dev_only_bytes ? dev_only_bytes : in_bytes + out_bytes;
  if (pp.dev_bytes < dev_need) {
    pp.dev_bytes = 0;
    for (int k = 0; k < kPipeSlots; ++k) {
      if (pp.dev[k]) { void* q = pp.dev[k]; pp.dev[k] = nullptr; HIP_TRY(hipFree(q)); }
      HIP_TRY(hipMalloc(&pp.dev[k], dev_need));
    }
    pp.dev_bytes = dev_need;
  }
  return GP_OK;
}

template <typename T>
static int64_t slab_rows(const gp_ctx* ctx, const gp_model* m, int64_t M, int64_t out_row_elems, int64_t max_rows) {
  constexpr int64_t kRowsPerWG = gpk::Geo<T>::kRowsPerWG;
  static const int rounds = [] { const char* ev = getenv("GP_HOST_SLAB_ROUNDS"); const int v = ev ? atoi(ev) : 2; return v < 1 ? 1 : v; }();
  int64_t slab = rounds * (int64_t)ctx->compute_units * gpk::Geo<T>::kWGPerCU * kRowsPerWG;
  const int64_t by_bytes = ((int64_t)(m->n_emulators > 1 ? 64 : 16) << 20) / (int64_t)(out_row_elems * sizeof(T));
  if (slab > by_bytes) slab = by_bytes;
  if (M < 4 * slab && M >= 4 * 8192) slab = (M + 3) / 4;
  slab = (slab + kRowsPerWG - 1) / kRowsPerWG * kRowsPerWG;
  if (max_rows > 0 && slab > max_rows) slab = max_rows;
  if (slab > M) slab = M;
  return slab < 1 ? 1 : slab;
}

template <typename T, typename FIn, typename FLaunch, typename FOut>
static int run_slab_pipeline(gp_ctx* ctx, int64_t M, int64_t slab, size_t in_row, size_t out_row,
                             FIn copy_in, FLaunch launch, FOut copy_out) {
  const size_t in_elems = (size_t)slab * in_row, out_elems = (size_t)slab * out_row;
  int rc = ensure_pipe(ctx, in_elems * sizeof(T), out_elems * sizeof(T));
  if (rc) return rc;
  gp_pipe& pp = ctx->pipe;
  const int64_t ns = (M + slab - 1) / slab;
  auto rows_of = [&](int64_t s) { return (s + 1) * slab <= M ? slab : M - s * slab; };
  auto tasks_for = [&](int64_t n, size_t row_bytes) {
    const size_t bytes = (size_t)n * row_bytes;
    int t = (int)(bytes / ((size_t)256 << 10));
    const int cap = 2 * host_threads();
    return t < 1 ? 1 : (t > cap ? cap : t);
  };
  static const bool trace = [] { const char* ev = getenv("GP_HOST_TRACE"); return ev && atoi(ev) != 0; }();
  auto now = [] { return std::chrono::steady_clock::now(); };
  double t_wait = 0, t_copy = 0, t_enq = 0;
  const auto t_begin = now();
  hipError_t e = hipSuccess;
  for (int64_t s = 0; s < ns + kPipeSlots && e == hipSuccess && rc == GP_OK; ++s) {
    const int k = (int)(s % kPipeSlots);
    const int64_t so = s - kPipeSlots;
    const bool has_out = so >= 0 && so < ns, has_in = s < ns;
    if (!has_out && !has_in) continue;
    const int64_t n_out = has_out ? rows_of(so) : 0, n_in = has_in ? rows_of(s) : 0;
    auto t0 = now();
    if (has_out) {
      e = hipEventSynchronize(pp.done[k]);
      if (e != hipSuccess) break;
    }
    auto t1 = now();
    const int t_out = has_out ? tasks_for(n_out, out_row * sizeof(T)) : 0;
    const int t_in = has_in ? tasks_for(n_in, in_row * sizeof(T)) : 0;
    const T* o_stage = (const T*)pp.stage_out[k];
    T* i_stage = (T*)pp.stage_in[k];
    auto task = [&](int t) {
      if (t < t_in) {
        const int64_t lo = n_in * t / t_in, hi = n_in * (t + 1) / t_in;
        copy_in(i_stage, s * slab, n_in, lo, hi);
      } else {
        const int u = t - t_in;
        const int64_t lo = n_out * u / t_out, hi = n_out * (u + 1) / t_out;
        copy_out(o_stage, so * slab, n_out, lo, hi);
      }
    };
    const int n_tasks = t_in + t_out;
    static const int skip_host = [] { const char* ev = getenv("GP_HOST_SKIP"); return ev ? atoi(ev) & 8 : 0; }();
    if (skip_host) {}
    else if (n_tasks == 1) task(0);
    else host_pool(ctx).run(n_tasks, task);
    auto t2 = now();
    if (has_in) {
      static const int skip = [] { const char* ev = getenv("GP_HOST_SKIP"); return ev ? atoi(ev) : 0; }();
      T* d_in = (T*)pp.dev[k];
      T* d_out = d_in + in_elems;
      static const int dir_streams = [] { const char* ev = getenv("GP_PIPE_DIRSTREAMS"); return ev ? atoi(ev) : 3; }();
      const bool own_up = dir_streams & 1, own_down = dir_streams & 2;
      hipStream_t s_up = own_up ? pp.up : pp.stream[k], s_down = own_down ? pp.down : pp.stream[k];
      if (!(skip & 1))
        e = hipMemcpyAsync(d_in, pp.stage_in[k], sizeof(T) * (size_t)n_in * in_row, hipMemcpyHostToDevice, s_up);
      if (e != hipSuccess) break;
      if (own_up) {
        e = hipEventRecord(pp.in_there[k], s_up);
        if (e == hipSuccess) e = hipStreamWaitEvent(pp.stream[k], pp.in_there[k], 0);
        if (e != hipSuccess) break;
      }
      if (!(skip & 2)) rc = launch(d_in, d_out, n_in, pp.stream[k]);
      if (rc) break;
      if (own_down) {
        e = hipEventRecord(pp.computed[k], pp.stream[k]);
        if (e == hipSuccess) e = hipStreamWaitEvent(s_down, pp.computed[k], 0);
        if (e != hipSuccess) break;
      }
      if (!(skip & 4))
        e = hipMemcpyAsync(pp.stage_out[k], d_out, sizeof(T) * (size_t)n_in * out_row, hipMemcpyDeviceToHost, s_down);
      if (e == hipSuccess) e = hipEventRecord(pp.done[k], s_down);
    }
    if (trace) {
      auto t3 = now();
      t_wait += std::chrono::duration<double>(t1 - t0).count();
      t_copy += std::chrono::duration<double>(t2 - t1).count();
      t_enq += std::chrono::duration<double>(t3 - t2).count();
    }
  }
  for (int k = 0; k < kPipeSlots; ++k) (void)hipStreamSynchronize(pp.stream[k]);
  (void)hipStreamSynchronize(pp.up);
  (void)hipStreamSynchronize(pp.down);
  if (trace)
    fprintf(stderr, "[gp host pipeline] rows=%lld slab=%lld slabs=%lld threads=%d: total %.3f ms = event waits %.3f + host copies %.3f + enqueue %.3f\n",
            (long long)M, (long long)slab, (long long)ns, host_threads(),
            std::chrono::duration<double>(now() - t_begin).count() * 1e3, t_wait * 1e3, t_copy * 1e3, t_enq * 1e3);
  if (rc) return rc;
  if (e != hipSuccess) return fail(GP_ERR_HIP, "host pipeline: %s", hipGetErrorString(e));
  return GP_OK;
}

static bool is_pinned_host(const void* p, size_t bytes) {
  if (!p) return false;
  hipPointerAttribute_t a;
  if (hipPointerGetAttributes(&a, p) != hipSuccess) { (void)hipGetLastError(); return false; }
  if (a.type != hipMemoryTypeHost) return false;
  hipPointerAttribute_t b;
  if (hipPointerGetAttributes(&b, (const char*)p + (bytes ? bytes - 1 : 0)) != hipSuccess) { (void)hipGetLastError(); return false; }
  return b.type == hipMemoryTypeHost;
}

template <typename T>
static int predict_host_pinned(gp_ctx* ctx, const gp_model* m, const T* testing, T* result, T* error, T* deriv,
                               int64_t M, int64_t max_rows) {
  const int D = m->n_inputs;
  constexpr int64_t kRowsPerWG = gpk::Geo<T>::kRowsPerWG;
  const int64_t round = (int64_t)ctx->compute_units * gpk::Geo<T>::kWGPerCU * kRowsPerWG;
  int64_t cap = 4 * round;
  if (max_rows > 0 && cap > max_rows) cap = max_rows < kRowsPerWG ? kRowsPerWG : max_rows / kRowsPerWG * kRowsPerWG;
  const bool want_var = error != nullptr;
  const size_t in_elems = (size_t)cap * D, out_elems = (size_t)cap * ((want_var ? 2 : 1) + D);
  int rc = ensure_pipe(ctx, 0, 0, (in_elems + out_elems) * sizeof(T));
  if (rc) return rc;
  gp_pipe& pp = ctx->pipe;
  hipError_t e = hipSuccess;
  int64_t s0 = 0, cur = round < cap ? round : cap;
  for (int64_t s = 0; s0 < M && e == hipSuccess && rc == GP_OK; ++s) {
    const int k = (int)(s % kPipeSlots);
    const int64_t n = s0 + cur <= M ? cur : M - s0;
    if (s >= kPipeSlots) e = hipEventSynchronize(pp.done[k]);
    if (e != hipSuccess) break;
    T* d_in = (T*)pp.dev[k];
    T* d_mu = d_in + in_elems;
    T* d_var = want_var ? d_mu + n : nullptr;
    T* d_der = d_mu + (want_var ? 2 : 1) * n;
    e = hipMemcpyAsync(d_in, testing + (size_t)s0 * D, sizeof(T) * (size_t)n * D, hipMemcpyHostToDevice, pp.up);
    if (e == hipSuccess) e = hipEventRecord(pp.in_there[k], pp.up);
    if (e == hipSuccess) e = hipStreamWaitEvent(pp.stream[k], pp.in_there[k], 0);
    if (e != hipSuccess) break;
    rc = predict_device<T>(ctx, m, d_in, d_mu, d_var, d_der, n, GP_DERIV_ROWMAJOR, pp.stream[k]);
    if (rc) break;
    e = hipEventRecord(pp.computed[k], pp.stream[k]);
    if (e == hipSuccess) e = hipStreamWaitEvent(pp.down, pp.computed[k], 0);
    if (e == hipSuccess) e = hipMemcpyAsync(deriv + (size_t)s0 * D, d_der, sizeof(T) * (size_t)n * D, hipMemcpyDeviceToHost, pp.down);
    if (e == hipSuccess) e = hipMemcpyAsync(result + s0, d_mu, sizeof(T) * (size_t)n, hipMemcpyDeviceToHost, pp.down);
    if (e == hipSuccess && want_var) e = hipMemcpyAsync(error + s0, d_var, sizeof(T) * (size_t)n, hipMemcpyDeviceToHost, pp.down);
    if (e == hipSuccess) e = hipEventRecord(pp.done[k], pp.down);
    s0 += n;
    if (2 * cur <= cap) cur *= 2;
  }
  for (int k = 0; k < kPipeSlots; ++k) (void)hipStreamSynchronize(pp.stream[k]);
  (void)hipStreamSynchronize(pp.up);
  (void)hipStreamSynchronize(pp.down);
  if (rc) return rc;
  if (e != hipSuccess) return fail(GP_ERR_HIP, "host pipeline (pinned arrays): %s", hipGetErrorString(e));
  return GP_OK;
}

template <typename T, typename TH>
static int predict_host(gp_ctx* ctx, const gp_model* m, const TH* testing, TH* result, TH* error,
                        TH* deriv, int64_t M, int layout, int64_t max_rows) {
  const int D = m->n_inputs, E = m->n_emulators;
  if (M == 0) return GP_OK;
  HIP_TRY(hipSetDevice(ctx->device));
  const bool want_var = error != nullptr;
  const int nv = want_var ? 2 : 1;
  const size_t out_row = (size_t)E * (nv + D);
  static const int64_t direct_rows = [] { const char* ev = getenv("GP_HOST_DIRECT_ROWS"); return ev ? (int64_t)atoll(ev) : (int64_t)32768; }();
  if (sizeof(T) == sizeof(TH) && M <= direct_rows && (max_rows <= 0 || M <= max_rows) &&
      (size_t)M * out_row * sizeof(T) <= ((size_t)32 << 20)) {
    const size_t n_in = (size_t)M * D, n_e = (size_t)E * M;
    int rc = ensure_scratch(ctx, (n_in + n_e * (nv + D)) * sizeof(T));
    if (rc) return rc;
    hipStream_t st = ctx->stream;
    T* d_in = (T*)ctx->scratch;
    T* d_mu = d_in + n_in;
    T* d_var = want_var ? d_mu + n_e : nullptr;
    T* d_der = d_mu + nv * n_e;
    HIP_TRY(hipMemcpyAsync(d_in, testing, n_in * sizeof(T), hipMemcpyHostToDevice, st));
    rc = predict_device<T>(ctx, m, d_in, d_mu, d_var, d_der, M, layout, st);
    hipError_t e = hipSuccess;
    if (!rc) {
      const bool one = want_var ? (const void*)error == (const void*)(result + n_e) && (const void*)deriv == (const void*)(error + n_e)
                                : (const void*)deriv == (const void*)(result + n_e);
      e = hipMemcpyAsync(result, d_mu, (one ? n_e * (nv + D) : n_e) * sizeof(T), hipMemcpyDeviceToHost, st);
      if (!one && want_var && e == hipSuccess) e = hipMemcpyAsync(error, d_var, n_e * sizeof(T), hipMemcpyDeviceToHost, st);
      if (!one && e == hipSuccess) e = hipMemcpyAsync(deriv, d_der, n_e * D * sizeof(T), hipMemcpyDeviceToHost, st);
    }
    const hipError_t es = hipStreamSynchronize(st);
    if (rc) return rc;
    if (e != hipSuccess || es != hipSuccess)
      return fail(GP_ERR_HIP, "predict (direct copies): %s", hipGetErrorString(e != hipSuccess ? e : es));
    return GP_OK;
  }
  if constexpr (sizeof(T) == sizeof(TH)) {
    static const bool no_pinned = [] { const char* ev = getenv("GP_NO_PINNED_PATH"); return ev && atoi(ev) != 0; }();
    if (!no_pinned && E == 1 && layout == GP_DERIV_ROWMAJOR &&
        is_pinned_host(testing, (size_t)M * D * sizeof(T)) && is_pinned_host(result, (size_t)M * sizeof(T)) &&
        (!want_var || is_pinned_host(error, (size_t)M * sizeof(T))) && is_pinned_host(deriv, (size_t)M * D * sizeof(T)))
      return predict_host_pinned<T>(ctx, m, (const T*)testing, (T*)result, (T*)error, (T*)deriv, M, max_rows);
  }
  const int64_t slab = slab_rows<T>(ctx, m, M, (int64_t)out_row, max_rows);
  const bool prescale = sizeof(T) == 4 && sizeof(TH) == 8 && E == 1 && m->kernel_nb > 0;
  const double* sc = m->scale_host.data();
  const double* ce = m->centre_host.data();
  auto copy_in = [=](T* stage, int64_t s0, int64_t n, int64_t lo, int64_t hi) {
    (void)n;
    const TH* src = testing + (size_t)s0 * D;
    if (prescale) {
      double sc8[8 * GP_MAX_KERNEL_D], ce8[8 * GP_MAX_KERNEL_D];
      for (int q = 0; q < 8 * D; ++q) { sc8[q] = sc[q % D]; ce8[q] = ce[q % D]; }
      int64_t r = lo;
      for (; r + 8 <= hi; r += 8) {
        const TH* a = src + (size_t)r * D;
        T* o = stage + (size_t)r * D;
        for (int q = 0; q < 8 * D; ++q) o[q] = (T)(sc8[q] * ((double)a[q] - ce8[q]));
      }
      for (; r < hi; ++r)
        for (int d = 0; d < D; ++d)
          stage[(size_t)r * D + d] = (T)(sc[d] * ((double)src[(size_t)r * D + d] - ce[d]));
    } else {
      convert_range(stage, src, (size_t)lo * D, (size_t)hi * D);
    }
  };
  auto launch = [=](T* d_in, T* d_out, int64_t n, hipStream_t st) {
    return predict_device<T>(ctx, m, d_in, d_out, want_var ? d_out + (size_t)E * n : nullptr, d_out + (size_t)nv * E * n, n,
                             layout, st, prescale);
  };
  auto copy_out = [=](const T* o, int64_t s0, int64_t n, int64_t lo, int64_t hi) {
    int e_lo = 0, e_hi = E;
    if (E > 1) {
      e_lo = (int)((int64_t)E * lo / n);
      e_hi = (int)((int64_t)E * hi / n);
      lo = 0;
      hi = n;
    }
    for (int e = e_lo; e < e_hi; ++e) {
      convert_range(result + (size_t)e * M + s0, o + (size_t)e * n, (size_t)lo, (size_t)hi);
      if (want_var) convert_range(error + (size_t)e * M + s0, o + (size_t)(E + e) * n, (size_t)lo, (size_t)hi);
      const T* od = o + (size_t)nv * E * n + (size_t)e * n * D;
      TH* hd = deriv + (size_t)e * M * D;
      if (layout == GP_DERIV_ROWMAJOR) {
        convert_range(hd + (size_t)s0 * D, od, (size_t)lo * D, (size_t)hi * D);
      } else {
        for (int d = 0; d < D; ++d)
          convert_range(hd + (size_t)d * M + s0, od + (size_t)d * n, (size_t)lo, (size_t)hi);
      }
    }
  };
  return run_slab_pipeline<T>(ctx, M, slab, (size_t)D, out_row, copy_in, launch, copy_out);
}

template <typename T, typename TH = T>
static int hessian_host_model(gp_ctx* ctx, const gp_model* m, const TH* testing, TH* hess, int64_t M) {
  const int D = m->n_inputs, E = m->n_emulators;
  if (M == 0) return GP_OK;
  HIP_TRY(hipSetDevice(ctx->device));
  const size_t dd = (size_t)D * D;
  const size_t out_row = (size_t)E * dd;
  if (sizeof(T) == sizeof(TH) && (size_t)M * out_row * sizeof(T) <= ((size_t)8 << 20)) {
    const size_t n_in = (size_t)M * D, n_out = (size_t)M * out_row;
    int rc = ensure_scratch(ctx, (n_in + n_out) * sizeof(T));
    if (rc) return rc;
    hipStream_t st = ctx->stream;
    T* d_in = (T*)ctx->scratch;
    T* d_out = d_in + n_in;
    HIP_TRY(hipMemcpyAsync(d_in, testing, n_in * sizeof(T), hipMemcpyHostToDevice, st));
    rc = hessian_device<T>(ctx, m, d_in, d_out, M, st);
    hipError_t e = hipSuccess;
    if (!rc) e = hipMemcpyAsync(hess, d_out, n_out * sizeof(T), hipMemcpyDeviceToHost, st);
    const hipError_t es = hipStreamSynchronize(st);
    if (rc) return rc;
    if (e != hipSuccess || es != hipSuccess)
      return fail(GP_ERR_HIP, "hessian (direct copies): %s", hipGetErrorString(e != hipSuccess ? e : es));
    return GP_OK;
  }
  const int64_t slab = slab_rows<T>(ctx, m, M, (int64_t)out_row, 0);
  auto copy_in = [=](T* stage, int64_t s0, int64_t, int64_t lo, int64_t hi) {
    convert_range(stage, testing + (size_t)s0 * D, (size_t)lo * D, (size_t)hi * D);
  };
  auto launch = [=](T* d_in, T* d_out, int64_t n, hipStream_t st) {
    return hessian_device<T>(ctx, m, d_in, d_out, n, st);
  };
  auto copy_out = [=](const T* o, int64_t s0, int64_t n, int64_t lo, int64_t hi) {
    int e_lo = 0, e_hi = 1;
    if (E > 1) {
      e_lo = (int)((int64_t)E * lo / n);
      e_hi = (int)((int64_t)E * hi / n);
      lo = 0;
      hi = n;
    }
    for (int e = e_lo; e < e_hi; ++e)
      convert_range(hess + ((size_t)e * M + s0) * dd, o + (size_t)e * n * dd, (size_t)lo * dd, (size_t)hi * dd);
  };
  return run_slab_pipeline<T>(ctx, M, slab, (size_t)D, out_row, copy_in, launch, copy_out);
}

template <typename T, typename TH = T>
static int predict_wrap(gp_ctx* ctx, const TH* expX, const TH* inputs, const TH* invQt,
                        const TH* invQ, const TH* testing, TH* result, TH* error, TH* deriv,
                        int64_t M, int N, int D, int theta_size, int layout = GP_DERIV_DMAJOR) {
  if (!ctx) return fail(GP_ERR_INVALID, "null context");
  if (M < 0) return fail(GP_ERR_INVALID, "n_predict < 0");
  if (M > 0 && (!testing || !result || !error || !deriv)) return fail(GP_ERR_INVALID, "null pointer");
  if (!invQ) return fail(GP_ERR_INVALID, "null pointer");
  HIP_TRY(hipSetDevice(ctx->device));
  gp_model* m = nullptr;
  int rc = cached_model<T, TH>(ctx, expX, inputs, invQt, invQ, N, D, theta_size, &m);
  if (rc) return rc;
  return predict_host<T, TH>(ctx, m, testing, result, error, deriv, M, layout, 0);
}

template <typename T>
static int hessian_host(gp_ctx* ctx, const T* expX, const T* inputs, const T* invQt,
                        const T* testing, T* hess, int64_t M, int N, int D, int theta_size) {
  if (!ctx) return fail(GP_ERR_INVALID, "null context");
  if (M < 0) return fail(GP_ERR_INVALID, "n_predict < 0");
  if (M > 0 && (!testing || !hess)) return fail(GP_ERR_INVALID, "null pointer");
  HIP_TRY(hipSetDevice(ctx->device));
  gp_model* m = nullptr;
  int rc = cached_model<T, T>(ctx, expX, inputs, invQt, (const T*)nullptr, N, D, theta_size, &m);
  if (rc) return rc;
  if ((rc = check_hessian_inputs(m->n_inputs))) return rc;
  return hessian_host_model<T>(ctx, m, testing, hess, M);
}

extern "C" {

static int predict_host_entry(gp_ctx* ctx, const gp_model* model, int host_dtype, const void* testing, void* result,
                              void* error, void* deriv, int64_t n_predict, int deriv_layout, int64_t max_block_rows,
                              bool want_var) {
  int rc = check_call(ctx, model, n_predict);
  if (rc || n_predict == 0) return rc;
  if (!testing || !result || (want_var && !error) || !deriv) return fail(GP_ERR_INVALID, "null pointer");
  if ((rc = check_layout(deriv_layout)) || (rc = check_model(ctx, model, want_var ? kNeedVariance : 0))) return rc;
  return guarded([&] { return for_dtypes(model->dtype, host_dtype, [&](auto t, auto th) {
    using TH = GP_TAG_TYPE(th);
    return predict_host<GP_TAG_TYPE(t), TH>(ctx, model, as<TH>(testing), as<TH>(result), as<TH>(error), as<TH>(deriv),
                                            n_predict, deriv_layout, max_block_rows);
  }); });
}
int gp_predict_mean_grad_host(gp_ctx* ctx, const gp_model* model, int host_dtype, const void* testing,
                              void* result, void* deriv, int64_t n_predict, int deriv_layout,
                              int64_t max_block_rows) {
  return predict_host_entry(ctx, model, host_dtype, testing, result, nullptr, deriv, n_predict, deriv_layout, max_block_rows, false);
}
int gp_predict_host(gp_ctx* ctx, const gp_model* model, int host_dtype, const void* testing,
                    void* result, void* error, void* deriv, int64_t n_predict, int deriv_layout,
                    int64_t max_block_rows) {
  return predict_host_entry(ctx, model, host_dtype, testing, result, error, deriv, n_predict, deriv_layout, max_block_rows, true);
}

static int hessian_host_entry(gp_ctx* ctx, const gp_model* model, int host_dtype, const void* testing, void* hess,
                              int64_t n_predict) {
  int rc = check_call(ctx, model, n_predict);
  if (rc || n_predict == 0) return rc;
  if (!testing || !hess) return fail(GP_ERR_INVALID, "null pointer");
  if ((rc = check_model(ctx, model, kNeedHessian))) return rc;
  return guarded([&] { return for_dtypes(model->dtype, host_dtype < 0 ? model->dtype : host_dtype, [&](auto t, auto th) {
    using TH = GP_TAG_TYPE(th);
    return hessian_host_model<GP_TAG_TYPE(t), TH>(ctx, model, as<TH>(testing), as<TH>(hess), n_predict);
  }); });
}
int gp_hessian_host(gp_ctx* ctx, const gp_model* model, const void* testing, void* hess, int64_t n_predict) {
  return hessian_host_entry(ctx, model, -1, testing, hess, n_predict);
}
int gp_hessian_host_h64(gp_ctx* ctx, const gp_model* model, const double* testing, double* hess, int64_t n_predict) {
  return hessian_host_entry(ctx, model, GP_F64, testing, hess, n_predict);
}

int gp_device_numa_node(int device, int* node) {
  if (!node) return fail(GP_ERR_INVALID, "null pointer");
  *node = device_numa_node(device);
  return GP_OK;
}

int gp_ctx_host_threads(gp_ctx* ctx, int* n_threads) {
  if (!ctx || !n_threads) return fail(GP_ERR_INVALID, "null pointer");
  *n_threads = host_threads();
  return GP_OK;
}

int gp_predict_wrap_f64(gp_ctx* ctx, const double* expX, const double* inputs, const double* invQt,
                        const double* invQ, const double* testing, double* result, double* error,
                        double* deriv, int64_t n_predict, int n_train, int n_inputs, int theta_size) {
  return guarded([&] { return predict_wrap<double>(ctx, expX, inputs, invQt, invQ, testing, result, error, deriv,
                              n_predict, n_train, n_inputs, theta_size); });
}
int gp_predict_wrap_f32(gp_ctx* ctx, const float* expX, const float* inputs, const float* invQt,
                        const float* invQ, const float* testing, float* result, float* error,
                        float* deriv, int64_t n_predict, int n_train, int n_inputs, int theta_size) {
  return guarded([&] { return predict_wrap<float>(ctx, expX, inputs, invQt, invQ, testing, result, error, deriv,
                             n_predict, n_train, n_inputs, theta_size); });
}

int gp_hessian_f64(gp_ctx* ctx, const double* expX, const double* inputs, const double* invQt,
                   const double* testing, double* hess, int64_t n_predict, int n_train,
                   int n_inputs, int theta_size) {
  return guarded([&] { return hessian_host<double>(ctx, expX, inputs, invQt, testing, hess, n_predict, n_train, n_inputs, theta_size); });
}
int gp_hessian_f32(gp_ctx* ctx, const float* expX, const float* inputs, const float* invQt,
                   const float* testing, float* hess, int64_t n_predict, int n_train,
                   int n_inputs, int theta_size) {
  return guarded([&] { return hessian_host<float>(ctx, expX, inputs, invQt, testing, hess, n_predict, n_train, n_inputs, theta_size); });
}

int gp_predict_rows_f64(gp_ctx* ctx, const double* expX, const double* inputs, const double* invQt,
                        const double* invQ, const double* testing, double* result, double* error,
                        double* deriv, int64_t n_predict, int n_train, int n_inputs, int theta_size) {
  return guarded([&] { return predict_wrap<double>(ctx, expX, inputs, invQt, invQ, testing, result, error, deriv,
                              n_predict, n_train, n_inputs, theta_size, GP_DERIV_ROWMAJOR); });
}
int gp_predict_rows_f32_h64(gp_ctx* ctx, const double* expX, const double* inputs, const double* invQt,
                            const double* invQ, const double* testing, double* result, double* error,
                            double* deriv, int64_t n_predict, int n_train, int n_inputs, int theta_size) {
  return guarded([&] { return predict_wrap<float, double>(ctx, expX, inputs, invQt, invQ, testing, result, error, deriv,
                                     n_predict, n_train, n_inputs, theta_size, GP_DERIV_ROWMAJOR); });
}
int gp_predict_rows_f32(gp_ctx* ctx, const float* expX, const float* inputs, const float* invQt,
                        const float* invQ, const float* testing, float* result, float* error,
                        float* deriv, int64_t n_predict, int n_train, int n_inputs, int theta_size) {
  return guarded([&] { return predict_wrap<float>(ctx, expX, inputs, invQt, invQ, testing, result, error, deriv,
                             n_predict, n_train, n_inputs, theta_size, GP_DERIV_ROWMAJOR); });
}

}
```

gp_emulator_amd/csrc/gp_host_pool.hpp:

```cpp
#pragma once
#include <atomic>
#include <condition_variable>
#include <mutex>
#include <thread>
#include <type_traits>
#include <vector>

#include <pthread.h>
#include <sched.h>

#if defined(__x86_64__)
#include <immintrin.h>
#endif

namespace gph {

inline void cpu_relax() {
#if defined(__x86_64__)
  _mm_pause();
#endif
}

class ThreadPool {
 public:
  explicit ThreadPool(int n_threads, const cpu_set_t* cpus = nullptr) {
    const int workers = n_threads > 1 ? n_threads - 1 : 0;
    for (int i = 0; i < workers; ++i) {
      threads_.emplace_back([this] { worker(); });
      if (cpus) (void)pthread_setaffinity_np(threads_.back().native_handle(), sizeof(cpu_set_t), cpus);
    }
  }
  ~ThreadPool() {
    {
      std::lock_guard<std::mutex> lk(mu_);
      stop_ = true;
      gen_.fetch_add(1, std::memory_order_release);
    }
    cv_.notify_all();
    for (auto& t : threads_) t.join();
  }
  ThreadPool(const ThreadPool&) = delete;
  ThreadPool& operator=(const ThreadPool&) = delete;

  int size() const { return (int)threads_.size() + 1; }

  template <typename F>
  void run_on_worker(F&& f) {
    if (threads_.empty()) { f(); return; }
    Job job;
    auto body = [&](int) { f(); };
    job.call = [](void* ctx, int t) { (*static_cast<decltype(body)*>(ctx))(t); };
    job.ctx = &body;
    job.n = 1;
    {
      std::lock_guard<std::mutex> lk(mu_);
      job_ = &job;
      gen_.fetch_add(1, std::memory_order_release);
    }
    cv_.notify_all();
    while (job.done.load(std::memory_order_acquire) < 1) std::this_thread::yield();
    {
      std::lock_guard<std::mutex> lk(mu_);
      job_ = nullptr;
    }
    while (job.attached.load(std::memory_order_acquire) != 0) cpu_relax();
  }

  template <typename F>
  void run(int n_tasks, F&& fn) {
    if (n_tasks <= 0) return;
    if (threads_.empty() || n_tasks == 1) {
      for (int t = 0; t < n_tasks; ++t) fn(t);
      return;
    }
    Job job;
    job.call = [](void* ctx, int t) { (*static_cast<typename std::remove_reference<F>::type*>(ctx))(t); };
    job.ctx = &fn;
    job.n = n_tasks;
    {
      std::lock_guard<std::mutex> lk(mu_);
      job_ = &job;
      gen_.fetch_add(1, std::memory_order_release);
    }
    cv_.notify_all();
    work(job);
    while (job.done.load(std::memory_order_acquire) < n_tasks) cpu_relax();
    {
      std::lock_guard<std::mutex> lk(mu_);
      job_ = nullptr;
    }
    while (job.attached.load(std::memory_order_acquire) != 0) cpu_relax();
  }

 private:
  struct Job {
    void (*call)(void*, int) = nullptr;
    void* ctx = nullptr;
    int n = 0;
    std::atomic<int> next{0}, done{0}, attached{0};
  };

  static void work(Job& job) {
    for (;;) {
      const int t = job.next.fetch_add(1, std::memory_order_relaxed);
      if (t >= job.n) break;
      job.call(job.ctx, t);
      job.done.fetch_add(1, std::memory_order_release);
    }
  }

  void worker() {
    unsigned long long seen = 0;
    for (;;) {
      for (int i = 0; i < 16000 && gen_.load(std::memory_order_acquire) == seen; ++i) cpu_relax();
      Job* job = nullptr;
      {
        std::unique_lock<std::mutex> lk(mu_);
        cv_.wait(lk, [&] { return gen_.load(std::memory_order_acquire) != seen; });
        seen = gen_.load(std::memory_order_acquire);
        if (stop_) return;
        job = job_;
        if (job) job->attached.fetch_add(1, std::memory_order_acq_rel);
      }
      if (job) {
        work(*job);
        job->attached.fetch_sub(1, std::memory_order_acq_rel);
      }
    }
  }

  std::vector<std::thread> threads_;
  std::mutex mu_;
  std::condition_variable cv_;
  std::atomic<unsigned long long> gen_{0};
  Job* job_ = nullptr;
  bool stop_ = false;
};

}
```

include/gp_predict_hip.h:

```cpp
#ifndef GP_PREDICT_HIP_H
#define GP_PREDICT_HIP_H

#include <stdint.h>

#ifdef __cplusplus
extern "C" {
#endif

typedef enum gp_status {
  GP_OK = 0,
  GP_STALE = 1,
  GP_ERR_INVALID = -1,
  GP_ERR_HIP = -2,
  GP_ERR_NO_DEVICE = -3,
  GP_ERR_UNSUPPORTED = -4,
  GP_ERR_NOMEM = -5
} gp_status;

typedef enum gp_dtype { GP_F32 = 0, GP_F64 = 1 } gp_dtype;

#define GP_DERIV_DMAJOR 0
#define GP_DERIV_ROWMAJOR 1

typedef struct gp_ctx gp_ctx;
typedef struct gp_model gp_model;
typedef struct gp_event gp_event;

const char* gp_last_error_string(void);
const char* gp_version_string(void);
int gp_device_count(int* count);

int gp_ctx_create(int device, gp_ctx** out);
int gp_ctx_destroy(gp_ctx* ctx);
int gp_ctx_synchronize(gp_ctx* ctx);
int gp_ctx_set_debug_buffer(gp_ctx* ctx, void* d_buffer);
int gp_ctx_device_info(gp_ctx* ctx, int* compute_units, int64_t* hbm_bytes, char* name, int name_len);

int gp_predict_wrap_f64(gp_ctx* ctx, const double* expX, const double* inputs,
                        const double* invQt, const double* invQ, const double* testing,
                        double* result, double* error, double* deriv,
                        int64_t n_predict, int n_train, int n_inputs, int theta_size);
int gp_predict_wrap_f32(gp_ctx* ctx, const float* expX, const float* inputs,
                        const float* invQt, const float* invQ, const float* testing,
                        float* result, float* error, float* deriv,
                        int64_t n_predict, int n_train, int n_inputs, int theta_size);

int gp_predict_rows_f64(gp_ctx* ctx, const double* expX, const double* inputs,
                        const double* invQt, const double* invQ, const double* testing,
                        double* result, double* error, double* deriv,
                        int64_t n_predict, int n_train, int n_inputs, int theta_size);
int gp_predict_rows_f32(gp_ctx* ctx, const float* expX, const float* inputs,
                        const float* invQt, const float* invQ, const float* testing,
                        float* result, float* error, float* deriv,
                        int64_t n_predict, int n_train, int n_inputs, int theta_size);

int gp_predict_rows_f32_h64(gp_ctx* ctx, const double* expX, const double* inputs,
                            const double* invQt, const double* invQ, const double* testing,
                            double* result, double* error, double* deriv,
                            int64_t n_predict, int n_train, int n_inputs, int theta_size);

int gp_model_create_f64(gp_ctx* ctx, const double* expX, const double* inputs,
                        const double* invQt, const double* invQ,
                        int n_train, int n_inputs, int theta_size, gp_model** out);
int gp_model_create_f32(gp_ctx* ctx, const float* expX, const float* inputs,
                        const float* invQt, const float* invQ,
                        int n_train, int n_inputs, int theta_size, gp_model** out);
int gp_model_create_f32_h64(gp_ctx* ctx, const double* expX, const double* inputs,
                            const double* invQt, const double* invQ,
                            int n_train, int n_inputs, int theta_size, gp_model** out);
int gp_batch_create_f64(gp_ctx* ctx, int n_emulators, const double* expX, const double* inputs,
                        const double* invQt, const double* invQ,
                        int n_train, int n_inputs, int theta_size, gp_model** out);
int gp_batch_create_f32(gp_ctx* ctx, int n_emulators, const float* expX, const float* inputs,
                        const float* invQt, const float* invQ,
                        int n_train, int n_inputs, int theta_size, gp_model** out);
int gp_batch_create_f32_h64(gp_ctx* ctx, int n_emulators, const double* expX, const double* inputs,
                            const double* invQt, const double* invQ,
                            int n_train, int n_inputs, int theta_size, gp_model** out);
int gp_model_emulators(const gp_model* model, int* n_emulators);
int gp_model_destroy(gp_model* model);
int gp_model_info(const gp_model* model, int* dtype, int* n_train, int* n_inputs,
                  int* kernel_d, int* kernel_nb);

int gp_predict_device(gp_ctx* ctx, const gp_model* model, const void* d_testing,
                      void* d_mu, void* d_var, void* d_deriv, int64_t n_predict,
                      int deriv_layout);

int gp_predict_host(gp_ctx* ctx, const gp_model* model, int host_dtype, const void* testing,
                    void* result, void* error, void* deriv, int64_t n_predict, int deriv_layout,
                    int64_t max_block_rows);
int gp_predict_mean_grad_device(gp_ctx* ctx, const gp_model* model, const void* d_testing,
                                void* d_mu, void* d_deriv, int64_t n_predict, int deriv_layout);
int gp_predict_mean_grad_host(gp_ctx* ctx, const gp_model* model, int host_dtype, const void* testing,
                              void* result, void* deriv, int64_t n_predict, int deriv_layout,
                              int64_t max_block_rows);
int gp_predict_var_grad_device(gp_ctx* ctx, const gp_model* model, const void* d_testing,
                               void* d_var, void* d_dvar, int64_t n_predict, int deriv_layout);
int gp_model_var_grad_bytes(const gp_model* model, int64_t* bytes);
int gp_ctx_host_threads(gp_ctx* ctx, int* n_threads);
int gp_device_numa_node(int device, int* node);

int gp_hessian_device(gp_ctx* ctx, const gp_model* model, const void* d_testing,
                      void* d_hess, int64_t n_predict);
int gp_hessian_host(gp_ctx* ctx, const gp_model* model, const void* testing, void* hess,
                    int64_t n_predict);
int gp_hessian_host_h64(gp_ctx* ctx, const gp_model* model, const double* testing, double* hess,
                        int64_t n_predict);
int gp_hessian_weighted_device(gp_ctx* ctx, const gp_model* model, const void* d_testing,
                               const void* d_weights, void* d_out, int64_t n_predict);
int gp_hessian_weighted_host(gp_ctx* ctx, const gp_model* model, int host_dtype, const void* testing,
                             const void* weights, void* out, int64_t n_predict);
int gp_hessian_f64(gp_ctx* ctx, const double* expX, const double* inputs, const double* invQt,
                   const double* testing, double* hess,
                   int64_t n_predict, int n_train, int n_inputs, int theta_size);
int gp_hessian_f32(gp_ctx* ctx, const float* expX, const float* inputs, const float* invQt,
                   const float* testing, float* hess,
                   int64_t n_predict, int n_train, int n_inputs, int theta_size);

int gp_reconstruct_device(gp_ctx* ctx, int dtype, const void* d_basis, const void* d_coef,
                          void* d_out, int64_t n_rows, int n_pcs, int n_bands);

int gp_mv_predict_host(gp_ctx* ctx, const gp_model* model, const void* d_basis, const void* y,
                       int64_t n_rows, int n_bands, void* fwd, void* jac);

uint64_t gp_content_digest(const void* const* blocks, const int64_t* nbytes, int n_blocks);
int gp_mv_predict_host_checked(gp_ctx* ctx, const gp_model* model, const void* d_basis, const void* y,
                               int64_t n_rows, int n_bands, void* fwd, void* jac,
                               const void* const* blocks, const int64_t* nbytes, int n_blocks, uint64_t expected);

int gp_mv_misfit_device(gp_ctx* ctx, int dtype, const void* d_basis, const void* d_mu, const void* d_deriv,
                        const void* d_obs, int64_t obs_stride, const void* d_weights, int64_t weights_stride,
                        void* d_cost, void* d_coef, void* d_grad, int64_t n_rows, int n_pcs, int n_bands, int n_inputs);
int gp_mv_gauss_newton_device(gp_ctx* ctx, int dtype, const void* d_deriv, const void* d_A, void* d_gn, int64_t n_rows,
                              int n_pcs, int n_inputs);
int gp_mv_weight_gram_device(gp_ctx* ctx, int dtype, const void* d_basis, const void* d_weights, int64_t weights_stride,
                             void* d_gram, int64_t n_rows, int n_pcs, int n_bands);
int gp_mv_gauss_newton_rows_device(gp_ctx* ctx, int dtype, const void* d_deriv, const void* d_gram, int64_t gram_stride,
                                   void* d_gn, int64_t n_rows, int n_pcs, int n_inputs);
int gp_mv_misfit_unc_device(gp_ctx* ctx, int dtype, const void* d_cost0, const void* d_coef, const void* d_gram,
                            int64_t gram_stride, const void* d_var, const void* d_deriv, const void* d_dvar, void* d_cost,
                            void* d_grad, void* d_gn, void* d_ceff, void* d_geff, int64_t n_rows, int n_pcs, int n_inputs);
int gp_mv_misfit_host(gp_ctx* ctx, const gp_model* model, const void* d_basis, const void* y, int64_t y_stride,
                      const void* obs, int64_t obs_stride, const void* weights, int64_t weights_stride, const void* A,
                      int64_t n_rows, int n_bands, void* out);
int gp_mv_misfit_host_checked(gp_ctx* ctx, const gp_model* model, const void* d_basis, const void* y, int64_t y_stride,
                              const void* obs, int64_t obs_stride, const void* weights, int64_t weights_stride,
                              const void* A, int64_t n_rows, int n_bands, void* out, const void* const* blocks,
                              const int64_t* nbytes, int n_blocks, uint64_t expected);

int gp_band_misfit_device(gp_ctx* ctx, const gp_model* batch, const void* d_testing, const void* d_obs,
                          int64_t obs_estride, int64_t obs_mstride, const void* d_weights, int64_t w_estride,
                          int64_t w_mstride, void* d_cost, void* d_grad, void* d_wr, void* d_gn, void* d_hess,
                          int64_t n_rows);
int gp_band_misfit_host(gp_ctx* ctx, const gp_model* batch, int host_dtype, const void* testing, const void* obs,
                        int64_t obs_estride, int64_t obs_mstride, const void* weights, int64_t w_estride,
                        int64_t w_mstride, void* cost, void* grad, void* wr, void* gn, void* hess, int64_t n_rows);

int gp_band_misfit_unc_device(gp_ctx* ctx, const gp_model* batch, const void* d_testing, const void* d_obs,
                              int64_t obs_estride, int64_t obs_mstride, const void* d_weights, int64_t w_estride,
                              int64_t w_mstride, void* d_cost, void* d_grad, void* d_wr, void* d_weff, void* d_gn,
                              int64_t n_rows);

#define GP_DAMP_DIAGONAL 0
#define GP_DAMP_IDENTITY 1
int gp_newton_step_device(gp_ctx* ctx, int dtype, const void* d_x, const void* d_grad, const void* d_A,
                          const void* d_lambda, int damping, const void* d_prior_mean, const void* d_prior_prec,
                          const void* d_lo, const void* d_hi, void* d_step, void* d_trial, int32_t* d_status,
                          int64_t n_rows, int n_inputs);
int gp_lm_update_device(gp_ctx* ctx, int dtype, void* d_x, const void* d_trial, void* d_cost, const void* d_cost_trial,
                        void* d_grad, const void* d_grad_trial, void* d_A, const void* d_A_trial,
                        void* d_lambda, const int32_t* d_status, int32_t* d_state, int32_t* d_accepted,
                        const void* d_prior_mean, const void* d_prior_prec, double down, double up,
                        double lambda_min, double lambda_max, double ftol, double xtol,
                        int64_t n_rows, int n_inputs);

int gp_newton_step_rows_device(gp_ctx* ctx, int dtype, const void* d_x, const void* d_grad, const void* d_A,
                               const void* d_lambda, int damping, const void* d_prior_mean, const void* d_prior_prec,
                               const void* d_lo, const void* d_hi, void* d_step, void* d_trial, int32_t* d_status,
                               int64_t n_rows, int n_inputs, int64_t prior_mean_stride, int64_t prior_prec_stride);
int gp_lm_update_rows_device(gp_ctx* ctx, int dtype, void* d_x, const void* d_trial, void* d_cost,
                             const void* d_cost_trial, void* d_grad, const void* d_grad_trial, void* d_A,
                             const void* d_A_trial, void* d_lambda, const int32_t* d_status, int32_t* d_state,
                             int32_t* d_accepted, const void* d_prior_mean, const void* d_prior_prec, double down,
                             double up, double lambda_min, double lambda_max, double ftol, double xtol,
                             int64_t n_rows, int n_inputs, int64_t prior_mean_stride, int64_t prior_prec_stride);

int gp_posterior_cov_device(gp_ctx* ctx, int dtype, const void* d_A, const void* d_prior_prec,
                            void* d_cov, void* d_sigma, int32_t* d_status, int64_t n_rows, int n_inputs);
int gp_posterior_cov_rows_device(gp_ctx* ctx, int dtype, const void* d_A, const void* d_prior_prec,
                                 void* d_cov, void* d_sigma, int32_t* d_status, int64_t n_rows, int n_inputs,
                                 int64_t prior_prec_stride);

int gp_prior_propagate_device(gp_ctx* ctx, int dtype, const void* d_A, const void* d_prior_prec,
                              int64_t prior_prec_stride, const void* d_noise, int64_t noise_stride,
                              void* d_next_prec, int32_t* d_status, int64_t n_rows, int n_inputs);

int gp_rts_smooth_device(gp_ctx* ctx, int dtype, const void* d_A, const void* d_prior_prec,
                         int64_t prior_prec_stride, const void* d_noise, int64_t noise_stride,
                         const void* d_x, const void* d_x_next, const void* d_cov_next,
                         const void* d_lo, const void* d_hi, void* d_x_smooth, void* d_cov_smooth,
                         void* d_sigma_smooth, int32_t* d_status, int64_t n_rows, int n_inputs);

int gp_lut_search_device(gp_ctx* ctx, int dtype, const void* d_table, int64_t table_kstride, int64_t table_lstride,
                         const void* d_offset, const void* d_obs, int64_t obs_kstride, int64_t obs_mstride,
                         const void* d_weights, int64_t w_kstride, int64_t w_mstride, int32_t* d_index, void* d_cost,
                         int64_t n_rows, int64_t n_candidates, int n_terms, int n_best, int n_slices);
int gp_lut_search_geometry(int* rows_per_item, int* candidate_tile, int* term_chunk);

int gp_lut_search_pc_device(gp_ctx* ctx, int dtype, const void* d_table, int64_t table_pstride, int64_t table_lstride,
                            const void* d_offset, const void* d_c0, const void* d_j0, const void* d_g0,
                            const void* d_gram, int64_t gram_stride, const int32_t* d_status, int32_t* d_index,
                            void* d_cost, int64_t n_rows, int64_t n_candidates, int n_pcs, int n_best, int n_slices);
int gp_lut_search_pc_geometry(int dtype, int n_pcs, int* rows_per_item, int* candidate_tile, int* padded_pcs,
                              int* workgroups_per_cu);

int gp_mv_lut_prepare_device(gp_ctx* ctx, int dtype, const void* d_basis, const void* d_obs, int64_t obs_stride,
                             const void* d_weights, int64_t weights_stride, void* d_gram, int64_t gram_stride,
                             void* d_c0, void* d_j0, void* d_g0, int32_t* d_status, int64_t n_rows, int n_pcs,
                             int n_bands);

int gp_likelihood_batch_f64(gp_ctx* ctx, int n_sets, const double* theta, const double* inputs,
                            const double* targets, int targets_shared, int n_train, int n_inputs,
                            double* cost, double* grad, double* invQ, double* invQt);

int gp_sobol_batch_f64(gp_ctx* ctx, int n_emulators, const double* expX, const double* inputs, const double* invQt,
                       int n_train, int n_inputs, int n_boxes, const double* lo, const double* hi, int n_pairs,
                       const int32_t* pairs, double* mean, double* cov);

int gp_moments_batch_f64(gp_ctx* ctx, int n_emulators, const double* expX, const double* inputs, const double* invQt,
                         const double* invQ, int n_train, int n_inputs, int64_t n_rows, const double* mean_in,
                         const double* cov_in, int n_pairs, const int32_t* pairs, double* mean, double* egrad,
                         double* cov, double* evar, int32_t* info);

int gp_frag_index(int kernel_nb, int I, int J, int s);
int gp_kernel_ksteps(int n_train, int n_inputs, int* ksteps);
int gp_pack_sizes(int dtype, int n_train, int n_inputs, int* kernel_d, int* kernel_nb,
                  int64_t* xa_len, int64_t* frags_len);
#define GP_OP_PREDICT 0
#define GP_OP_MEAN_GRAD 1
#define GP_OP_HESSIAN 2
#define GP_OP_RECONSTRUCT 3
#define GP_OP_MISFIT 4
#define GP_OP_MV_GRAM 5
#define GP_OP_VAR_GRAD 6
#define GP_OP_LUT_SEARCH 7
#define GP_OP_LUT_SEARCH_PC 8
#define GP_OP_SOBOL 9
#define GP_OP_MOMENTS 10
#define GP_PLAN_PREDICT_FEW 1
#define GP_PLAN_PREDICT 2
#define GP_PLAN_GENERIC 3
#define GP_PLAN_HESS_VALU 4
#define GP_PLAN_HESS_WIN_KL3 5
#define GP_PLAN_HESS_WIN_KL4 6
#define GP_PLAN_HESS_WIN_DIRECT 7
#define GP_PLAN_RECON_NARROW 8
#define GP_PLAN_RECON_WIDE 9
#define GP_PLAN_MISFIT 10
#define GP_PLAN_MV_GRAM 11
#define GP_PLAN_VAR_GRAD 12
#define GP_PLAN_LUT_SEARCH 13
#define GP_PLAN_LUT_SEARCH_PC 14
#define GP_PLAN_SOBOL 15
#define GP_PLAN_MOMENTS 16
int gp_launch_plan(int op, int dtype, int n_train, int n_inputs, int n_emulators, int64_t n_rows, int aux,
                   int compute_units, int aligned16, int* kernel, int64_t* items, int* workgroups,
                   int64_t* rest_items, int* rest_workgroups, int* rows_per_item);
int gp_pack_model_f64(const double* expX, const double* inputs, const double* invQt,
                      const double* invQ, int n_train, int n_inputs, int theta_size,
                      double* xa, double* frags, double* sd, double* b);
int gp_pack_model_f32(const float* expX, const float* inputs, const float* invQt,
                      const float* invQ, int n_train, int n_inputs, int theta_size,
                      float* xa, float* frags, float* sd, float* b);

int gp_pinned_alloc(gp_ctx* ctx, int64_t bytes, void** ptr);
int gp_pinned_free(gp_ctx* ctx, void* ptr);

int gp_malloc(gp_ctx* ctx, int64_t bytes, void** dptr);
int gp_free(gp_ctx* ctx, void* dptr);
int gp_memcpy_h2d(gp_ctx* ctx, void* dst_device, const void* src_host, int64_t bytes);
int gp_memcpy_d2h(gp_ctx* ctx, void* dst_host, const void* src_device, int64_t bytes);
int gp_memset(gp_ctx* ctx, void* dptr, int value, int64_t bytes);
int gp_event_create(gp_ctx* ctx, gp_event** out);
int gp_event_destroy(gp_event* ev);
int gp_event_record(gp_ctx* ctx, gp_event* ev);
int gp_event_elapsed_ms(gp_event* start, gp_event* stop, float* ms);

#ifdef __cplusplus
}
#endif
#endif
```

Baseline: 770.5 million.

## Unify host slab pipeline with direct pinned copies and async output staging

Reworks the host slab pipeline so pinned inputs and outputs are copied straight to and from the device, skipping the staging buffers, while staged outputs are unpacked asynchronously on the thread pool and overlap later slabs. Slab sizes start small and double up to a cap so the first results arrive sooner. The output pool now allocates page-locked memory up to a budget, so returned arrays qualify for the direct path. This adds async pool machinery and more pinned memory use, and the finer-grained event handling brings some risk of contention or ordering bugs.

```diff
diff --git a/gp_emulator_amd/_lib.py b/gp_emulator_amd/_lib.py
--- a/gp_emulator_amd/_lib.py
+++ b/gp_emulator_amd/_lib.py
@@ -2,6 +2,7 @@
 import os
 import sys
 import threading
+import weakref
 
 import numpy as np
 
@@ -122,6 +123,7 @@
     "gp_pack_model_f32": (c_int, [c_void_p] * 4 + [c_int, c_int, c_int] + [c_void_p] * 4),
     "gp_pinned_alloc": (c_int, [c_void_p, c_i64, PP]),
     "gp_pinned_free": (c_int, [c_void_p, c_void_p]),
+    "gp_is_page_locked": (c_int, [c_void_p, c_i64, ctypes.POINTER(c_int)]),
     "gp_malloc": (c_int, [c_void_p, c_i64, PP]),
     "gp_free": (c_int, [c_void_p, c_void_p]),
     "gp_memcpy_h2d": (c_int, [c_void_p, c_void_p, c_void_p, c_i64]),
@@ -280,11 +282,34 @@
     return cpus
 
 
+def is_page_locked(a):
+    if not a.flags["C_CONTIGUOUS"]:
+        raise ValueError("a must be C-contiguous")
+    yes = c_int(0)
+    check(load().gp_is_page_locked(c_void_p(a.ctypes.data), a.nbytes, ctypes.byref(yes)), "gp_is_page_locked")
+    return bool(yes.value)
+
+
 class OutputPool:
 
-    def __init__(self, max_item=256 << 20, max_total=1 << 30):
+    def __init__(self, max_item=256 << 20, max_total=1 << 30, pinned_alloc=None, pinned_budget=None):
         self.max_item, self.max_total = max_item, max_total
         self.items = []
+        self.pinned_alloc = pinned_alloc
+        if pinned_budget is None:
+            pinned_budget = int(float(os.environ.get("GP_OUT_POOL_PINNED_MB", "512")) * (1 << 20))
+        self.pinned_budget = pinned_budget
+
+    def pinned_bytes(self):
+        return sum(b.nbytes for b in self.items if not b.flags["OWNDATA"])
+
+    def _fresh(self, nbytes):
+        if self.pinned_alloc is not None and self.pinned_bytes() + nbytes <= self.pinned_budget:
+            try:
+                return self.pinned_alloc(nbytes)
+            except GpuPredictError:
+                pass
+        return np.empty(nbytes, np.uint8)
 
     def take(self, shape, dtype):
         dtype = np.dtype(dtype)
@@ -298,7 +323,7 @@
                 break
         cand = None
         if base is None:
-            base = np.empty(nbytes, np.uint8)
+            base = self._fresh(nbytes)
             self.items.append(base)
             total = sum(b.nbytes for b in self.items)
             for free_first in (True, False):
@@ -353,20 +378,23 @@
             raise GpuPredictUnavailable("no usable GPU context on device %d: %s" % (device, msg))
         self.h = h
         self.device = int(device)
-        self.out_pool = OutputPool()
+        me = weakref.ref(self)
+        self.out_pool = OutputPool(pinned_alloc=lambda nbytes: me()._pinned_bytes(nbytes))
+
+    def _pinned_bytes(self, nbytes):
+        if not getattr(self, "h", None):
+            raise GpuPredictError("the context is closed")
+        ptr = c_void_p()
+        check(self.lib.gp_pinned_alloc(self.h, max(1, nbytes), ctypes.byref(ptr)), "gp_pinned_alloc")
+        buf = (ctypes.c_char * max(1, nbytes)).from_address(ptr.value)
+        lib, addr = self.lib, ptr.value
+        weakref.finalize(buf, lambda: lib.gp_pinned_free(None, c_void_p(addr)))
+        return np.frombuffer(buf, dtype=np.uint8, count=nbytes)
 
     def pinned_empty(self, shape, dtype=np.float64):
-        import weakref
         dtype = np.dtype(dtype)
         n = int(np.prod(shape, dtype=np.int64))
-        nbytes = max(1, n * dtype.itemsize)
-        ptr = c_void_p()
-        check(self.lib.gp_pinned_alloc(self.h, nbytes, ctypes.byref(ptr)), "gp_pinned_alloc")
-        buf = (ctypes.c_char * nbytes).from_address(ptr.value)
-        arr = np.frombuffer(buf, dtype=np.uint8, count=n * dtype.itemsize).view(dtype).reshape(shape)
-        lib, h, addr = self.lib, self.h, ptr.value
-        weakref.finalize(buf, lambda: lib.gp_pinned_free(h, c_void_p(addr)))
-        return arr
+        return self._pinned_bytes(n * dtype.itemsize).view(dtype).reshape(shape)
 
     def close(self):
         if getattr(self, "h", None):
diff --git a/gp_emulator_amd/csrc/gp_ctx.hip b/gp_emulator_amd/csrc/gp_ctx.hip
--- a/gp_emulator_amd/csrc/gp_ctx.hip
+++ b/gp_emulator_amd/csrc/gp_ctx.hip
@@ -212,10 +212,8 @@
   *ptr = q;
   return GP_OK;
 }
-int gp_pinned_free(gp_ctx* ctx, void* ptr) {
-  if (!ctx) return fail(GP_ERR_INVALID, "null context");
+int gp_pinned_free(gp_ctx*, void* ptr) {
   if (!ptr) return GP_OK;
-  HIP_TRY(hipSetDevice(ctx->device));
   HIP_TRY(hipHostFree(ptr));
   return GP_OK;
 }
diff --git a/gp_emulator_amd/csrc/gp_host_path.hip b/gp_emulator_amd/csrc/gp_host_path.hip
--- a/gp_emulator_amd/csrc/gp_host_path.hip
+++ b/gp_emulator_amd/csrc/gp_host_path.hip
@@ -1,4 +1,5 @@
 #include "gp_host.hpp"
+#include "gp_launch_plan.hpp"
 
 #include <cctype>
 #include <chrono>
@@ -66,7 +67,7 @@
   return *ctx->pipe.pool;
 }
 
-static int ensure_pipe(gp_ctx* ctx, size_t in_bytes, size_t out_bytes, size_t dev_only_bytes = 0) {
+static int ensure_pipe(gp_ctx* ctx, size_t in_bytes, size_t out_bytes, bool stage_in, bool stage_out) {
   gp_pipe& pp = ctx->pipe;
   if (!pp.ready) {
     for (int k = 0; k < kPipeSlots; ++k) {
@@ -89,7 +90,7 @@
     });
     return err;
   };
-  if (dev_only_bytes == 0 && pp.stage_in_bytes < in_bytes) {
+  if (stage_in && pp.stage_in_bytes < in_bytes) {
     pp.stage_in_bytes = 0;
     for (int k = 0; k < kPipeSlots; ++k) {
       if (pp.stage_in[k]) { void* q = pp.stage_in[k]; pp.stage_in[k] = nullptr; HIP_TRY(hipHostFree(q)); }
@@ -97,7 +98,7 @@
     }
     pp.stage_in_bytes = in_bytes;
   }
-  if (dev_only_bytes == 0 && pp.stage_out_bytes < out_bytes) {
+  if (stage_out && pp.stage_out_bytes < out_bytes) {
     pp.stage_out_bytes = 0;
     for (int k = 0; k < kPipeSlots; ++k) {
       if (pp.stage_out[k]) { void* q = pp.stage_out[k]; pp.stage_out[k] = nullptr; HIP_TRY(hipHostFree(q)); }
@@ -105,7 +106,7 @@
     }
     pp.stage_out_bytes = out_bytes;
   }
-  const size_t dev_need = dev_only_bytes ? dev_only_bytes : in_bytes + out_bytes;
+  const size_t dev_need = in_bytes + out_bytes;
   if (pp.dev_bytes < dev_need) {
     pp.dev_bytes = 0;
     for (int k = 0; k < kPipeSlots; ++k) {
@@ -131,98 +132,138 @@
   return slab < 1 ? 1 : slab;
 }
 
-template <typename T, typename FIn, typename FLaunch, typename FOut>
-static int run_slab_pipeline(gp_ctx* ctx, int64_t M, int64_t slab, size_t in_row, size_t out_row,
-                             FIn copy_in, FLaunch launch, FOut copy_out) {
-  const size_t in_elems = (size_t)slab * in_row, out_elems = (size_t)slab * out_row;
-  int rc = ensure_pipe(ctx, in_elems * sizeof(T), out_elems * sizeof(T));
+template <typename T, typename FIn, typename FLaunch, typename FOut, typename FDown>
+static int run_slab_pipeline(gp_ctx* ctx, int64_t M, int64_t first, int64_t cap, size_t in_row, size_t out_row,
+                             const T* rows_direct, bool out_direct, FIn copy_in, FLaunch launch, FOut copy_out,
+                             FDown download) {
+  const bool stage_in = rows_direct == nullptr, stage_out = !out_direct;
+  const size_t in_elems = (size_t)cap * in_row, out_elems = (size_t)cap * out_row;
+  int rc = ensure_pipe(ctx, in_elems * sizeof(T), out_elems * sizeof(T), stage_in, stage_out);
   if (rc) return rc;
   gp_pipe& pp = ctx->pipe;
-  const int64_t ns = (M + slab - 1) / slab;
-  auto rows_of = [&](int64_t s) { return (s + 1) * slab <= M ? slab : M - s * slab; };
+  const int slots = kPipeSlots;
+  gph::ThreadPool* pool = stage_in || stage_out ? &host_pool(ctx) : nullptr;
   auto tasks_for = [&](int64_t n, size_t row_bytes) {
     const size_t bytes = (size_t)n * row_bytes;
     int t = (int)(bytes / ((size_t)256 << 10));
-    const int cap = 2 * host_threads();
-    return t < 1 ? 1 : (t > cap ? cap : t);
+    const int cap_t = 2 * host_threads();
+    return t < 1 ? 1 : (t > cap_t ? cap_t : t);
   };
   static const bool trace = [] { const char* ev = getenv("GP_HOST_TRACE"); return ev && atoi(ev) != 0; }();
-  auto now = [] { return std::chrono::steady_clock::now(); };
+  static const int skip = [] { const char* ev = getenv("GP_HOST_SKIP"); return ev ? atoi(ev) : 0; }();
   double t_wait = 0, t_copy = 0, t_enq = 0;
-  const auto t_begin = now();
+  const auto t_begin = std::chrono::steady_clock::now();
+  auto t_last = t_begin;
+  auto lap = [&](double& acc) {
+    const auto t = std::chrono::steady_clock::now();
+    acc += std::chrono::duration<double>(t - t_last).count();
+    t_last = t;
+  };
+
+  struct OutJob {
+    FOut* f;
+    const T* stage;
+    int64_t s0, n;
+    int tasks;
+    void operator()(int t) { (*f)(stage, s0, n, n * t / tasks, n * (t + 1) / tasks); }
+  };
+  OutJob out_job[kPipeSlotsMax];
+  gph::ThreadPool::Handle out_h[kPipeSlotsMax];
+  bool out_pending[kPipeSlotsMax] = {};
+  int64_t ring_s0[kPipeSlotsMax] = {}, ring_n[kPipeSlotsMax] = {};
+  int64_t issued = 0;
+  int64_t out_next = 0;
+  auto submit_out = [&](int64_t so) {
+    const int k = (int)(so % slots);
+    out_job[k] = OutJob{&copy_out, (const T*)pp.stage_out[k], ring_s0[k], ring_n[k], tasks_for(ring_n[k], out_row * sizeof(T))};
+    if (skip & 8) return;
+    out_h[k] = pool->submit(out_job[k].tasks, out_job[k]);
+    out_pending[k] = true;
+  };
+  auto poll_out = [&]() -> hipError_t {
+    while (out_next < issued) {
+      const hipError_t q = hipEventQuery(pp.done[out_next % slots]);
+      if (q == hipErrorNotReady) { (void)hipGetLastError(); break; }
+      if (q != hipSuccess) return q;
+      submit_out(out_next++);
+    }
+    return hipSuccess;
+  };
+
   hipError_t e = hipSuccess;
-  for (int64_t s = 0; s < ns + kPipeSlots && e == hipSuccess && rc == GP_OK; ++s) {
-    const int k = (int)(s % kPipeSlots);
-    const int64_t so = s - kPipeSlots;
-    const bool has_out = so >= 0 && so < ns, has_in = s < ns;
-    if (!has_out && !has_in) continue;
-    const int64_t n_out = has_out ? rows_of(so) : 0, n_in = has_in ? rows_of(s) : 0;
-    auto t0 = now();
-    if (has_out) {
-      e = hipEventSynchronize(pp.done[k]);
+  int64_t s0 = 0, cur = first < cap ? first : cap;
+  while (s0 < M && e == hipSuccess && rc == GP_OK) {
+    const int64_t s = issued;
+    const int k = (int)(s % slots);
+    const int64_t n = s0 + cur <= M ? cur : M - s0;
+    T* d_in = (T*)pp.dev[k];
+    T* d_out = d_in + in_elems;
+    lap(t_enq);
+    if (stage_in) {
+      if (s >= slots) e = hipEventSynchronize(pp.in_there[k]);
       if (e != hipSuccess) break;
-    }
-    auto t1 = now();
-    const int t_out = has_out ? tasks_for(n_out, out_row * sizeof(T)) : 0;
-    const int t_in = has_in ? tasks_for(n_in, in_row * sizeof(T)) : 0;
-    const T* o_stage = (const T*)pp.stage_out[k];
-    T* i_stage = (T*)pp.stage_in[k];
-    auto task = [&](int t) {
-      if (t < t_in) {
-        const int64_t lo = n_in * t / t_in, hi = n_in * (t + 1) / t_in;
-        copy_in(i_stage, s * slab, n_in, lo, hi);
-      } else {
-        const int u = t - t_in;
-        const int64_t lo = n_out * u / t_out, hi = n_out * (u + 1) / t_out;
-        copy_out(o_stage, so * slab, n_out, lo, hi);
+      lap(t_wait);
+      T* i_stage = (T*)pp.stage_in[k];
+      const int t_in = tasks_for(n, in_row * sizeof(T));
+      auto task = [&](int t) { copy_in(i_stage, s0, n, n * t / t_in, n * (t + 1) / t_in); };
+      if (skip & 8) {}
+      else if (t_in == 1) task(0);
+      else pool->run(t_in, task);
+      lap(t_copy);
+    }
+    if (stage_out && (e = poll_out()) != hipSuccess) break;
+    if (s >= slots) e = hipStreamWaitEvent(pp.up, pp.computed[k], 0);
+    if (e == hipSuccess && !(skip & 1))
+      e = hipMemcpyAsync(d_in, stage_in ? (const T*)pp.stage_in[k] : rows_direct + (size_t)s0 * in_row,
+                         sizeof(T) * (size_t)n * in_row, hipMemcpyHostToDevice, pp.up);
+    if (e == hipSuccess) e = hipEventRecord(pp.in_there[k], pp.up);
+    if (e == hipSuccess) e = hipStreamWaitEvent(pp.stream[k], pp.in_there[k], 0);
+    if (e == hipSuccess && s >= slots) e = hipStreamWaitEvent(pp.stream[k], pp.done[k], 0);
+    if (e != hipSuccess) break;
+    if (!(skip & 2)) rc = launch(d_in, d_out, n, pp.stream[k]);
+    if (rc) break;
+    e = hipEventRecord(pp.computed[k], pp.stream[k]);
+    if (e == hipSuccess) e = hipStreamWaitEvent(pp.down, pp.computed[k], 0);
+    if (e != hipSuccess) break;
+    lap(t_enq);
+    if (stage_out && s >= slots) {
+      if (out_next <= s - slots) {
+        e = hipEventSynchronize(pp.done[k]);
+        if (e != hipSuccess) break;
+        lap(t_wait);
+        submit_out(out_next++);
       }
-    };
-    const int n_tasks = t_in + t_out;
-    static const int skip_host = [] { const char* ev = getenv("GP_HOST_SKIP"); return ev ? atoi(ev) & 8 : 0; }();
-    if (skip_host) {}
-    else if (n_tasks == 1) task(0);
-    else host_pool(ctx).run(n_tasks, task);
-    auto t2 = now();
-    if (has_in) {
-      static const int skip = [] { const char* ev = getenv("GP_HOST_SKIP"); return ev ? atoi(ev) : 0; }();
-      T* d_in = (T*)pp.dev[k];
-      T* d_out = d_in + in_elems;
-      static const int dir_streams = [] { const char* ev = getenv("GP_PIPE_DIRSTREAMS"); return ev ? atoi(ev) : 3; }();
-      const bool own_up = dir_streams & 1, own_down = dir_streams & 2;
-      hipStream_t s_up = own_up ? pp.up : pp.stream[k], s_down = own_down ? pp.down : pp.stream[k];
-      if (!(skip & 1))
-        e = hipMemcpyAsync(d_in, pp.stage_in[k], sizeof(T) * (size_t)n_in * in_row, hipMemcpyHostToDevice, s_up);
-      if (e != hipSuccess) break;
-      if (own_up) {
-        e = hipEventRecord(pp.in_there[k], s_up);
-        if (e == hipSuccess) e = hipStreamWaitEvent(pp.stream[k], pp.in_there[k], 0);
-        if (e != hipSuccess) break;
-      }
-      if (!(skip & 2)) rc = launch(d_in, d_out, n_in, pp.stream[k]);
-      if (rc) break;
-      if (own_down) {
-        e = hipEventRecord(pp.computed[k], pp.stream[k]);
-        if (e == hipSuccess) e = hipStreamWaitEvent(s_down, pp.computed[k], 0);
-        if (e != hipSuccess) break;
-      }
-      if (!(skip & 4))
-        e = hipMemcpyAsync(pp.stage_out[k], d_out, sizeof(T) * (size_t)n_in * out_row, hipMemcpyDeviceToHost, s_down);
-      if (e == hipSuccess) e = hipEventRecord(pp.done[k], s_down);
-    }
-    if (trace) {
-      auto t3 = now();
-      t_wait += std::chrono::duration<double>(t1 - t0).count();
-      t_copy += std::chrono::duration<double>(t2 - t1).count();
-      t_enq += std::chrono::duration<double>(t3 - t2).count();
-    }
-  }
-  for (int k = 0; k < kPipeSlots; ++k) (void)hipStreamSynchronize(pp.stream[k]);
+      if (out_pending[k]) { pool->wait(out_h[k]); out_pending[k] = false; }
+      lap(t_copy);
+    }
+    if (skip & 4) {}
+    else if (out_direct) e = download(d_out, s0, n, pp.down);
+    else e = hipMemcpyAsync(pp.stage_out[k], d_out, sizeof(T) * (size_t)n * out_row, hipMemcpyDeviceToHost, pp.down);
+    if (e == hipSuccess) e = hipEventRecord(pp.done[k], pp.down);
+    ring_s0[k] = s0;
+    ring_n[k] = n;
+    ++issued;
+    s0 += n;
+    if (2 * cur <= cap) cur *= 2;
+  }
+  lap(t_enq);
+  while (stage_out && out_next < issued && e == hipSuccess && rc == GP_OK) {
+    e = hipEventSynchronize(pp.done[out_next % slots]);
+    lap(t_wait);
+    if (e == hipSuccess) submit_out(out_next++);
+  }
+  for (int k = 0; k < slots; ++k)
+    if (out_pending[k]) pool->wait(out_h[k]);
+  lap(t_copy);
+  for (int k = 0; k < slots; ++k) (void)hipStreamSynchronize(pp.stream[k]);
   (void)hipStreamSynchronize(pp.up);
   (void)hipStreamSynchronize(pp.down);
+  lap(t_wait);
   if (trace)
-    fprintf(stderr, "[gp host pipeline] rows=%lld slab=%lld slabs=%lld threads=%d: total %.3f ms = event waits %.3f + host copies %.3f + enqueue %.3f\n",
-            (long long)M, (long long)slab, (long long)ns, host_threads(),
-            std::chrono::duration<double>(now() - t_begin).count() * 1e3, t_wait * 1e3, t_copy * 1e3, t_enq * 1e3);
+    fprintf(stderr, "[gp host pipeline] rows=%lld slab=%lld..%lld slabs=%lld threads=%d rows %s results %s: total %.3f ms = event waits %.3f + host copies %.3f + enqueue %.3f\n",
+            (long long)M, (long long)(first < cap ? first : cap), (long long)cap, (long long)issued, host_threads(),
+            stage_in ? "staged" : "direct", stage_out ? "staged" : "direct",
+            std::chrono::duration<double>(t_last - t_begin).count() * 1e3, t_wait * 1e3, t_copy * 1e3, t_enq * 1e3);
   if (rc) return rc;
   if (e != hipSuccess) return fail(GP_ERR_HIP, "host pipeline: %s", hipGetErrorString(e));
   return GP_OK;
@@ -233,57 +274,21 @@
   hipPointerAttribute_t a;
   if (hipPointerGetAttributes(&a, p) != hipSuccess) { (void)hipGetLastError(); return false; }
   if (a.type != hipMemoryTypeHost) return false;
-  hipPointerAttribute_t b;
-  if (hipPointerGetAttributes(&b, (const char*)p + (bytes ? bytes - 1 : 0)) != hipSuccess) { (void)hipGetLastError(); return false; }
-  return b.type == hipMemoryTypeHost;
-}
-
-template <typename T>
-static int predict_host_pinned(gp_ctx* ctx, const gp_model* m, const T* testing, T* result, T* error, T* deriv,
-                               int64_t M, int64_t max_rows) {
-  const int D = m->n_inputs;
-  constexpr int64_t kRowsPerWG = gpk::Geo<T>::kRowsPerWG;
-  const int64_t round = (int64_t)ctx->compute_units * gpk::Geo<T>::kWGPerCU * kRowsPerWG;
-  int64_t cap = 4 * round;
-  if (max_rows > 0 && cap > max_rows) cap = max_rows < kRowsPerWG ? kRowsPerWG : max_rows / kRowsPerWG * kRowsPerWG;
-  const bool want_var = error != nullptr;
-  const size_t in_elems = (size_t)cap * D, out_elems = (size_t)cap * ((want_var ? 2 : 1) + D);
-  int rc = ensure_pipe(ctx, 0, 0, (in_elems + out_elems) * sizeof(T));
-  if (rc) return rc;
-  gp_pipe& pp = ctx->pipe;
-  hipError_t e = hipSuccess;
-  int64_t s0 = 0, cur = round < cap ? round : cap;
-  for (int64_t s = 0; s0 < M && e == hipSuccess && rc == GP_OK; ++s) {
-    const int k = (int)(s % kPipeSlots);
-    const int64_t n = s0 + cur <= M ? cur : M - s0;
-    if (s >= kPipeSlots) e = hipEventSynchronize(pp.done[k]);
-    if (e != hipSuccess) break;
-    T* d_in = (T*)pp.dev[k];
-    T* d_mu = d_in + in_elems;
-    T* d_var = want_var ? d_mu + n : nullptr;
-    T* d_der = d_mu + (want_var ? 2 : 1) * n;
-    e = hipMemcpyAsync(d_in, testing + (size_t)s0 * D, sizeof(T) * (size_t)n * D, hipMemcpyHostToDevice, pp.up);
-    if (e == hipSuccess) e = hipEventRecord(pp.in_there[k], pp.up);
-    if (e == hipSuccess) e = hipStreamWaitEvent(pp.stream[k], pp.in_there[k], 0);
-    if (e != hipSuccess) break;
-    rc = predict_device<T>(ctx, m, d_in, d_mu, d_var, d_der, n, GP_DERIV_ROWMAJOR, pp.stream[k]);
-    if (rc) break;
-    e = hipEventRecord(pp.computed[k], pp.stream[k]);
-    if (e == hipSuccess) e = hipStreamWaitEvent(pp.down, pp.computed[k], 0);
-    if (e == hipSuccess) e = hipMemcpyAsync(deriv + (size_t)s0 * D, d_der, sizeof(T) * (size_t)n * D, hipMemcpyDeviceToHost, pp.down);
-    if (e == hipSuccess) e = hipMemcpyAsync(result + s0, d_mu, sizeof(T) * (size_t)n, hipMemcpyDeviceToHost, pp.down);
-    if (e == hipSuccess && want_var) e = hipMemcpyAsync(error + s0, d_var, sizeof(T) * (size_t)n, hipMemcpyDeviceToHost, pp.down);
-    if (e == hipSuccess) e = hipEventRecord(pp.done[k], pp.down);
-    s0 += n;
-    if (2 * cur <= cap) cur *= 2;
-  }
-  for (int k = 0; k < kPipeSlots; ++k) (void)hipStreamSynchronize(pp.stream[k]);
-  (void)hipStreamSynchronize(pp.up);
-  (void)hipStreamSynchronize(pp.down);
-  if (rc) return rc;
-  if (e != hipSuccess) return fail(GP_ERR_HIP, "host pipeline (pinned arrays): %s", hipGetErrorString(e));
-  return GP_OK;
-}
+  void* base = nullptr;
+  size_t size = 0;
+  hipDeviceptr_t q = const_cast<void*>(p);
+  if (hipPointerGetAttribute(&base, HIP_POINTER_ATTRIBUTE_RANGE_START_ADDR, q) != hipSuccess ||
+      hipPointerGetAttribute(&size, HIP_POINTER_ATTRIBUTE_RANGE_SIZE, q) != hipSuccess) {
+    (void)hipGetLastError();
+    return false;
+  }
+  const char* lo = (const char*)base;
+  const char* first = (const char*)p;
+  return lo != nullptr && first >= lo && bytes <= size && (size_t)(first - lo) <= size - bytes;
+}
+
+constexpr int kMaxDirectCopies = 16;
+
 
 template <typename T, typename TH>
 static int predict_host(gp_ctx* ctx, const gp_model* m, const TH* testing, TH* result, TH* error,
@@ -321,14 +326,26 @@
       return fail(GP_ERR_HIP, "predict (direct copies): %s", hipGetErrorString(e != hipSuccess ? e : es));
     return GP_OK;
   }
+  const T* rows_direct = nullptr;
+  bool out_direct = false;
   if constexpr (sizeof(T) == sizeof(TH)) {
     static const bool no_pinned = [] { const char* ev = getenv("GP_NO_PINNED_PATH"); return ev && atoi(ev) != 0; }();
-    if (!no_pinned && E == 1 && layout == GP_DERIV_ROWMAJOR &&
-        is_pinned_host(testing, (size_t)M * D * sizeof(T)) && is_pinned_host(result, (size_t)M * sizeof(T)) &&
-        (!want_var || is_pinned_host(error, (size_t)M * sizeof(T))) && is_pinned_host(deriv, (size_t)M * D * sizeof(T)))
-      return predict_host_pinned<T>(ctx, m, (const T*)testing, (T*)result, (T*)error, (T*)deriv, M, max_rows);
-  }
-  const int64_t slab = slab_rows<T>(ctx, m, M, (int64_t)out_row, max_rows);
+    const size_t n_e = (size_t)E * M;
+    if (!no_pinned && is_pinned_host(testing, (size_t)M * D * sizeof(T))) rows_direct = (const T*)testing;
+    out_direct = !no_pinned && (int64_t)E * (nv + (layout == GP_DERIV_ROWMAJOR ? 1 : D)) <= kMaxDirectCopies &&
+                 is_pinned_host(result, n_e * sizeof(T)) && (!want_var || is_pinned_host(error, n_e * sizeof(T))) &&
+                 is_pinned_host(deriv, n_e * D * sizeof(T));
+  }
+  int64_t slab_first, slab_cap;
+  if (rows_direct && out_direct && E == 1) {
+    constexpr int64_t kRowsPerWG = gpk::Geo<T>::kRowsPerWG;
+    const int64_t round = (int64_t)ctx->compute_units * gpk::Geo<T>::kWGPerCU * kRowsPerWG;
+    slab_cap = 4 * round;
+    if (max_rows > 0 && slab_cap > max_rows) slab_cap = max_rows < kRowsPerWG ? kRowsPerWG : max_rows / kRowsPerWG * kRowsPerWG;
+    slab_first = round < slab_cap ? round : slab_cap;
+  } else {
+    slab_first = slab_cap = slab_rows<T>(ctx, m, M, (int64_t)out_row, max_rows);
+  }
   const bool prescale = sizeof(T) == 4 && sizeof(TH) == 8 && E == 1 && m->kernel_nb > 0;
   const double* sc = m->scale_host.data();
   const double* ce = m->centre_host.data();
@@ -351,9 +368,10 @@
       convert_range(stage, src, (size_t)lo * D, (size_t)hi * D);
     }
   };
+  const bool few_call = gpk::plan_predict_few(gpk::plan_grid(M, gpk::kTile, E, (int64_t)0x7fffffff).items, ctx->compute_units);
   auto launch = [=](T* d_in, T* d_out, int64_t n, hipStream_t st) {
     return predict_device<T>(ctx, m, d_in, d_out, want_var ? d_out + (size_t)E * n : nullptr, d_out + (size_t)nv * E * n, n,
-                             layout, st, prescale);
+                             layout, st, prescale, 0, -1, few_call);
   };
   auto copy_out = [=](const T* o, int64_t s0, int64_t n, int64_t lo, int64_t hi) {
     int e_lo = 0, e_hi = E;
@@ -376,7 +394,29 @@
       }
     }
   };
-  return run_slab_pipeline<T>(ctx, M, slab, (size_t)D, out_row, copy_in, launch, copy_out);
+  auto download = [=](const T* o, int64_t s0, int64_t n, hipStream_t st) -> hipError_t {
+    T* h_mu = (T*)(void*)result;
+    T* h_var = (T*)(void*)error;
+    T* h_der = (T*)(void*)deriv;
+    hipError_t err = hipSuccess;
+    auto down = [&](T* dst, const T* src, size_t count) {
+      if (err == hipSuccess) err = hipMemcpyAsync(dst, src, sizeof(T) * count, hipMemcpyDeviceToHost, st);
+    };
+    for (int e = 0; e < E; ++e) {
+      const T* od = o + (size_t)nv * E * n + (size_t)e * n * D;
+      T* hd = h_der + (size_t)e * M * D;
+      if (layout == GP_DERIV_ROWMAJOR) {
+        down(hd + (size_t)s0 * D, od, (size_t)n * D);
+      } else {
+        for (int d = 0; d < D; ++d) down(hd + (size_t)d * M + s0, od + (size_t)d * n, (size_t)n);
+      }
+      down(h_mu + (size_t)e * M + s0, o + (size_t)e * n, (size_t)n);
+      if (want_var) down(h_var + (size_t)e * M + s0, o + (size_t)(E + e) * n, (size_t)n);
+    }
+    return err;
+  };
+  return run_slab_pipeline<T>(ctx, M, slab_first, slab_cap, (size_t)D, out_row, rows_direct, out_direct, copy_in, launch,
+                              copy_out, download);
 }
 
 template <typename T, typename TH = T>
@@ -421,7 +461,9 @@
     for (int e = e_lo; e < e_hi; ++e)
       convert_range(hess + ((size_t)e * M + s0) * dd, o + (size_t)e * n * dd, (size_t)lo * dd, (size_t)hi * dd);
   };
-  return run_slab_pipeline<T>(ctx, M, slab, (size_t)D, out_row, copy_in, launch, copy_out);
+  auto download = [](const T*, int64_t, int64_t, hipStream_t) { return hipSuccess; };
+  return run_slab_pipeline<T>(ctx, M, slab, slab, (size_t)D, out_row, (const T*)nullptr, false, copy_in, launch, copy_out,
+                              download);
 }
 
 template <typename T, typename TH = T>
@@ -503,6 +545,12 @@
   return GP_OK;
 }
 
+int gp_is_page_locked(const void* ptr, int64_t bytes, int* yes) {
+  if (!yes || bytes < 0) return fail(GP_ERR_INVALID, "null pointer");
+  *yes = is_pinned_host(ptr, (size_t)bytes) ? 1 : 0;
+  return GP_OK;
+}
+
 int gp_ctx_host_threads(gp_ctx* ctx, int* n_threads) {
   if (!ctx || !n_threads) return fail(GP_ERR_INVALID, "null pointer");
   *n_threads = host_threads();
diff --git a/gp_emulator_amd/csrc/gp_host_pool.hpp b/gp_emulator_amd/csrc/gp_host_pool.hpp
--- a/gp_emulator_amd/csrc/gp_host_pool.hpp
+++ b/gp_emulator_amd/csrc/gp_host_pool.hpp
@@ -92,6 +92,63 @@
     while (job.attached.load(std::memory_order_acquire) != 0) cpu_relax();
   }
 
+  static constexpr int kAsyncSlots = 8;
+  struct Handle { int slot = -1; };
+
+  template <typename F>
+  Handle submit(int n_tasks, F& fn) {
+    Handle h;
+    if (n_tasks <= 0) return h;
+    if (!threads_.empty()) {
+      std::lock_guard<std::mutex> lk(mu_);
+      for (int i = 0; i < kAsyncSlots && h.slot < 0; ++i)
+        if (!async_[i].used) h.slot = i;
+      if (h.slot >= 0) {
+        Async& a = async_[h.slot];
+        a.call = [](void* ctx, int t) { (*static_cast<F*>(ctx))(t); };
+        a.ctx = &fn;
+        a.n = n_tasks;
+        a.next = 0;
+        a.done.store(0, std::memory_order_relaxed);
+        a.used = true;
+        gen_.fetch_add(1, std::memory_order_release);
+      }
+    }
+    if (h.slot < 0) {
+      for (int t = 0; t < n_tasks; ++t) fn(t);
+      return h;
+    }
+    cv_.notify_all();
+    return h;
+  }
+  bool finished(Handle h) {
+    if (h.slot < 0) return true;
+    std::lock_guard<std::mutex> lk(mu_);
+    const Async& a = async_[h.slot];
+    return a.done.load(std::memory_order_acquire) >= a.n;
+  }
+  void wait(Handle h) {
+    if (h.slot < 0) return;
+    Async& a = async_[h.slot];
+    int n = 0;
+    for (;;) {
+      void (*call)(void*, int) = nullptr;
+      void* ctx = nullptr;
+      int t = -1;
+      {
+        std::lock_guard<std::mutex> lk(mu_);
+        n = a.n;
+        if (a.next < a.n) { t = a.next++; call = a.call; ctx = a.ctx; }
+      }
+      if (t < 0) break;
+      call(ctx, t);
+      a.done.fetch_add(1, std::memory_order_release);
+    }
+    while (a.done.load(std::memory_order_acquire) < n) cpu_relax();
+    std::lock_guard<std::mutex> lk(mu_);
+    a.used = false;
+  }
+
  private:
   struct Job {
     void (*call)(void*, int) = nullptr;
@@ -99,6 +156,34 @@
     int n = 0;
     std::atomic<int> next{0}, done{0}, attached{0};
   };
+  struct Async {
+    void (*call)(void*, int) = nullptr;
+    void* ctx = nullptr;
+    int n = 0, next = 0;
+    std::atomic<int> done{0};
+    bool used = false;
+  };
+
+  void drain_async() {
+    for (;;) {
+      Async* a = nullptr;
+      void (*call)(void*, int) = nullptr;
+      void* ctx = nullptr;
+      int t = -1;
+      {
+        std::lock_guard<std::mutex> lk(mu_);
+        if (job_ && job_->next.load(std::memory_order_relaxed) < job_->n) return;
+        for (int i = 0; i < kAsyncSlots && !a; ++i)
+          if (async_[i].used && async_[i].next < async_[i].n) a = &async_[i];
+        if (!a) return;
+        t = a->next++;
+        call = a->call;
+        ctx = a->ctx;
+      }
+      call(ctx, t);
+      a->done.fetch_add(1, std::memory_order_release);
+    }
+  }
 
   static void work(Job& job) {
     for (;;) {
@@ -126,6 +211,7 @@
         work(*job);
         job->attached.fetch_sub(1, std::memory_order_acq_rel);
       }
+      drain_async();
     }
   }
 
@@ -134,6 +220,7 @@
   std::condition_variable cv_;
   std::atomic<unsigned long long> gen_{0};
   Job* job_ = nullptr;
+  Async async_[kAsyncSlots];
   bool stop_ = false;
 };
 
diff --git a/include/gp_predict_hip.h b/include/gp_predict_hip.h
--- a/include/gp_predict_hip.h
+++ b/include/gp_predict_hip.h
@@ -275,6 +275,7 @@
 
 int gp_pinned_alloc(gp_ctx* ctx, int64_t bytes, void** ptr);
 int gp_pinned_free(gp_ctx* ctx, void* ptr);
+int gp_is_page_locked(const void* ptr, int64_t bytes, int* yes);
 
 int gp_malloc(gp_ctx* ctx, int64_t bytes, void** dptr);
 int gp_free(gp_ctx* ctx, void* dptr);
```

After: 770.3 million. About the same (-0.0%).
